# facebookresearch/SlowFast

Measured on AMD Instinct MI355X. Metric: clips/sec (fwd+bwd), SlowFast-8x8-R50 32x224^2 synthetic clips, per-GPU batch 32, higher is better.
Workload: dtype fp16; 1 GPU; SLOWFAST_8x8_R50: forward + cross_entropy loss + backward + sgd step, inputs resident in HBM, per-GPU batch 32; global_batch=32, parallelism=dp1, launch=hip-graph(fwd+bwd) + eager all-reduce/optimizer, optimizer=FlatOptimizer (fused unscale+norm+clip+update, dynamic loss scale on device)

## Files before the change

include/sfamd.h:

```cpp
#ifndef SFAMD_H
#define SFAMD_H
#include <stddef.h>
#include <stdint.h>
#ifdef __cplusplus
extern "C" {
#endif

#define SF_ABI_VERSION 32
typedef void* sf_stream_t;

typedef struct sf_conv_desc {
    int32_t N, Ci, Ti, Hi, Wi;
    int32_t Co, To, Ho, Wo;
    int32_t kT, kH, kW;
    int32_t sT, sH, sW;
    int32_t pT, pH, pW;
    int32_t dT, dH, dW;
    int32_t Cw;
    int32_t ldx, ldy;
    int32_t Cow;
} sf_conv_desc;

int sf_abi_version(void);
const char* sf_backend(void);
#define SF_ACT_FP16 0
#define SF_ACT_BF16_ID 1
int sf_act_dtype(void);
const char* sf_last_error(void);
const char* sf_build_id(void);

int sf_conv_weight_ld(const sf_conv_desc* d, int32_t* ldf, int32_t* ldd);
int sf_prep_weights(const sf_conv_desc* d, const float* w, void* wf, void* wd, sf_stream_t stream);
typedef struct sf_prep_item {
    const float* w;
    void* wf;
    void* wd;
    int32_t Co, Cow, Cw, Cp, taps, ldf, ldd;
    int32_t pad;
} sf_prep_item;
int sf_prep_item_fill(const sf_conv_desc* d, const float* w, void* wf, void* wd, sf_prep_item* item);
int64_t sf_prep_item_blocks(const sf_prep_item* item);
int sf_prep_weights_batch(const sf_prep_item* items, const int32_t* blk_item, const int32_t* blk_off, int32_t nblocks,
                          sf_stream_t stream);
int sf_conv_fwd_mtiles(const sf_conv_desc* d);
int sf_conv_fwd(const sf_conv_desc* d, const void* x, const void* wf, const float* in_scale, const float* in_shift,
                int in_relu, const float* bias, void* y, float* stat_part, sf_stream_t stream);
int sf_conv_fwd_fused(const sf_conv_desc* d, const void* x, const void* wf, const float* bias, const void* resid,
                      int32_t ldr, int out_relu, void* y, sf_stream_t stream);
int sf_conv_dgrad(const sf_conv_desc* d, const void* dy, const void* wd, const void* resid, int32_t ldr,
                  const void* resid_bits, void* dx, sf_stream_t stream);
int sf_conv_dgrad_bn(const sf_conv_desc* d, const void* dy, const void* wd, const void* resid, int32_t ldr,
                     const void* resid_bits, void* dx, const float* mask_scale, const float* mask_shift,
                     const void* mask_bits, const void* bn_y, int32_t bn_ldy, float* bn_part, int32_t bn_part_rows,
                     int32_t* bn_rows, sf_stream_t stream);
int64_t sf_conv_wgrad_workspace(const sf_conv_desc* d);
int64_t sf_conv_wgrad_rowtab_bytes(const sf_conv_desc* d);
int sf_conv_wgrad_rowtab(const sf_conv_desc* d, void* tab, sf_stream_t stream);
int sf_conv_wgrad(const sf_conv_desc* d, const void* x, const float* in_scale, const float* in_shift, int in_relu,
                  const void* dy, float* dw, float out_scale, int zero_first, void* workspace, int64_t workspace_bytes,
                  const void* rowtab, sf_stream_t stream);
int sf_conv_c_bwd_plan(const sf_conv_desc* d, int in_affine, int mask_bits, int32_t* tile_rows, int64_t* workspace_bytes);
int sf_conv_c_bwd(const sf_conv_desc* d, const void* dz, int32_t lddz, const void* mask_bits, const void* yc, int32_t ldyc,
                  const float* coef, const void* act, const void* wd, const float* bn_scale, const float* bn_shift,
                  const void* bn_y, int32_t bn_ldy, float* bn_part, int32_t bn_part_rows, int32_t* bn_rows, void* d_in,
                  int32_t ld_in, float* dw, float out_scale, int zero_first, void* workspace, int64_t workspace_bytes,
                  sf_stream_t stream);

int sf_bn_finalize(float* part, int32_t nblk, int32_t C, int32_t Creal, float count, const float* gamma, const float* beta,
                   float* running_mean, float* running_var, float momentum, float eps, float* scale, float* shift,
                   float* save_mean, float* save_rstd, sf_stream_t stream);
int sf_bn_act(int64_t M, int32_t C, const void* y, int32_t ldy, const float* scale, const float* shift, const void* r,
              int32_t ldr, const float* rscale, const float* rshift, int relu, void* out, int32_t ldo, void* mask_out,
              sf_stream_t stream);
int sf_bn_bwd_blocks(int64_t M, int32_t C);
int sf_bn_bwd_reduce(int64_t M, int32_t C, const void* dz, int32_t lddz, const void* zmask, int32_t ldm, const void* y,
                     int32_t ldy, const float* scale, const float* shift, int relu_self, float* part,
                     sf_stream_t stream);
int sf_bn_bwd_finalize(float* part, int32_t nblk, int32_t C, int32_t Creal, float count, const float* gamma, const float* mean,
                       const float* rstd, float inv_loss_scale, float* dgamma, float* dbeta, int accumulate,
                       float* coef, sf_stream_t stream);
int sf_bn_bwd_apply(int64_t M, int32_t C, const void* dz, int32_t lddz, const void* zmask, int32_t ldm, const void* y,
                    int32_t ldy, const float* scale, const float* shift, int relu_self, const float* coef, void* dy,
                    int32_t lddy, void* gout, int32_t ldg, sf_stream_t stream);

int sf_pool_fwd(int32_t N, int32_t T, int32_t H, int32_t W, int32_t C, int32_t kH, int32_t kW, int32_t sH, int32_t sW,
                int32_t pH, int32_t pW, const void* y, int32_t ldy, const float* scale, const float* shift, int relu,
                void* out, int32_t ldo, void* argmax, int32_t cls, sf_stream_t stream);
int sf_pool_bwd(int32_t N, int32_t T, int32_t H, int32_t W, int32_t C, int32_t kH, int32_t kW, int32_t sH, int32_t sW,
                int32_t pH, int32_t pW, const void* pooled, int32_t ldp, const void* argmax, int relu,
                const void* dout, int32_t lddo, void* g, int32_t ldg, int32_t cls, sf_stream_t stream);

int sf_pool3d_fwd(int32_t N, int32_t T, int32_t H, int32_t W, int32_t C, int32_t kT, int32_t kH, int32_t kW, const void* x,
                  int32_t ldx, void* out, int32_t ldo, void* argmax, sf_stream_t stream);
int sf_pool3d_bwd(int32_t N, int32_t T, int32_t H, int32_t W, int32_t C, int32_t kT, int32_t kH, int32_t kW,
                  const void* argmax, const void* dout, int32_t lddo, void* dx, int32_t lddx, sf_stream_t stream);

int sf_ncthw_to_cl(const float* x, int32_t N, int32_t C, int64_t S, int32_t Cp, void* out, sf_stream_t stream);
int sf_cl_to_ncthw(const void* x, int32_t ld, int32_t N, int32_t C, int64_t S, float* out, sf_stream_t stream);


int sf_bgemm(int64_t M, int32_t N, int32_t K, const void* A, int32_t lda, const void* W, int32_t ldw, const float* bias,
             const void* resid, int32_t ldr, void* Y, int32_t ldy, int32_t nbatch, int32_t bh, int64_t sa_b, int64_t sa_h,
             int64_t sw_b, int64_t sw_h, int64_t sy_b, int64_t sy_h, int64_t sr_b, int64_t sr_h, int32_t resid_row0,
             float alpha, sf_stream_t stream);
typedef struct sf_rows32 {
    const float* in;
    float* out;
    int32_t ld, period;
} sf_rows32;
int sf_gemm_rows32(int64_t M, int32_t N, int32_t K, const void* A, int32_t lda, const void* W, int32_t ldw, const float* bias,
                   const void* resid, int32_t ldr, void* Y, int32_t ldy, const sf_rows32* side, sf_stream_t stream);
int sf_bgemm_tn(int64_t M, int32_t R, int32_t Kc, const void* P, int32_t ldp, const void* X, int32_t ldx, void* Out,
                int32_t ldo, float scale, int32_t nbatch, int32_t bh, int64_t sp_b, int64_t sp_h, int64_t sx_b,
                int64_t sx_h, int64_t so_b, int64_t so_h, sf_stream_t stream);

int sf_layernorm_fwd(int64_t M, int32_t C, const void* x, int32_t ldx, const float* gamma, const float* beta, float eps,
                     void* y, int32_t ldy, float* mean, float* rstd, sf_stream_t stream);
int sf_layernorm_fwd_rows32(int64_t M, int32_t C, const void* x, int32_t ldx, const float* gamma, const float* beta, float eps,
                            void* y, int32_t ldy, float* mean, float* rstd, const sf_rows32* side, sf_stream_t stream);
int sf_layernorm_bwd_blocks(int64_t M, int32_t C);
int sf_layernorm_bwd(int64_t M, int32_t C, const void* dy, int32_t lddy, const void* x, int32_t ldx, const float* gamma,
                     const float* mean, const float* rstd, const void* resid, int32_t ldr, void* dx, int32_t lddx,
                     float* part, sf_stream_t stream);
int sf_layernorm_bwd_sums(int64_t M, int32_t C, const void* dy, int32_t lddy, const void* x, int32_t ldx, const float* gamma,
                          const float* mean, const float* rstd, const void* resid, int32_t ldr, void* dx, int32_t lddx,
                          float* part, sf_stream_t stream);
int sf_colsum_blocks(int64_t M, int32_t C);
int sf_colsum(int64_t M, int32_t C, const void* x, int32_t ldx, float* part, sf_stream_t stream);
int sf_colsum_finalize(float* part, int32_t nblk, int32_t C, int32_t fold, float* out0, float* out1, float scale,
                       int accumulate, sf_stream_t stream);
typedef struct sf_colfin_item {
    float* part;
    int32_t nblk, C, fold;
    float* out0;
    float* out1;
    float scale;
    int32_t accumulate;
    int32_t row_stride;
} sf_colfin_item;
int sf_colsum_finalize_batch(const sf_colfin_item* items, int32_t n, sf_stream_t stream);
int sf_rows_sum(const float* part, int32_t nblk, int64_t row_len, int64_t offset, int32_t n, float* out, float scale,
                int accumulate, sf_stream_t stream);
int sf_gelu_fwd(int64_t n, const void* h, void* a, sf_stream_t stream);
int sf_gelu_bwd(int64_t n, const void* h, const void* da, void* dh, sf_stream_t stream);

typedef struct sf_dw_desc {
    int32_t N, C, Cw, cls;
    int32_t Ti, Hi, Wi, To, Ho, Wo;
    int32_t kT, kH, kW, sT, sH, sW, pT, pH, pW;
    int32_t ldx, ldy;
    int32_t Cwreal;
} sf_dw_desc;
int sf_dwconv_fwd_blocks(const sf_dw_desc* d);
int sf_dwconv_fwd_sample_rows(const sf_dw_desc* d);
int sf_dwconv_fwd(const sf_dw_desc* d, const void* x, const float* w, void* y, float* stat_part, sf_stream_t stream);
int sf_dwconv_dgrad(const sf_dw_desc* d, const void* dy, const float* w, void* dx, sf_stream_t stream);
int sf_dwconv_dgrad_sum_rows(const sf_dw_desc* d);
int sf_dwconv_dgrad_sums(const sf_dw_desc* d, const void* dy, const float* w, void* dx, float* sum_part, sf_stream_t stream);
int64_t sf_dwconv_wgrad_workspace(const sf_dw_desc* d);
int sf_dwconv_wgrad(const sf_dw_desc* d, const void* x, const void* dy, float* dw, float out_scale, int zero_first,
                    void* workspace, int64_t workspace_bytes, sf_stream_t stream);
int sf_dwconv_pair_ok(const sf_dw_desc* d);
int sf_dwconv_fwd_pair(const sf_dw_desc* d, const void* x, const void* x2, const float* w, const float* w2, void* y, void* y2,
                       sf_stream_t stream);
int sf_dwconv_dgrad_pair(const sf_dw_desc* d, const void* dy, const void* dy2, const float* w, const float* w2, void* dx, void* dx2,
                         sf_stream_t stream);
int sf_dwconv_wgrad_pair(const sf_dw_desc* d, const void* x, const void* x2, const void* dy, const void* dy2, float* dw, float* dw2,
                         float out_scale, int zero_first, int zero_first2, void* workspace, int64_t workspace_bytes,
                         sf_stream_t stream);

typedef struct sf_attn_desc {
    int32_t B, heads, D, cls;
    int32_t Nq, qT, qH, qW;
    int32_t Nk, kT, kH, kW;
    int32_t rows_h, rows_w, rows_t;
} sf_attn_desc;
int sf_relpos_gather(const sf_attn_desc* d, const void* G, int32_t ldg, const int32_t* idx_h, const int32_t* idx_w,
                     const int32_t* idx_t, float* rq, sf_stream_t stream);
int sf_relpos_scatter(const sf_attn_desc* d, const float* drq, const int32_t* idx_h, const int32_t* idx_w,
                      const int32_t* idx_t, void* E, int32_t lde, sf_stream_t stream);
int sf_relpos_pack(const float* rel_h, const float* rel_w, const float* rel_t, int32_t rows_h, int32_t rows_w, int32_t rows_t,
                   int32_t D, int32_t TRp, void* t16, void* t16t, sf_stream_t stream);
int sf_relpos_unpack(const float* dtab, int32_t rows_h, int32_t rows_w, int32_t rows_t, int32_t D, float* grad_h, float* grad_w,
                     float* grad_t, int32_t acc_h, int32_t acc_w, int32_t acc_t, sf_stream_t stream);
int sf_softmax_fwd(const sf_attn_desc* d, void* s, int32_t lds, float scale, const float* rq, sf_stream_t stream);
int sf_softmax_bwd(const sf_attn_desc* d, void* dp, const void* prob, int32_t lds, float scale, float* drq,
                   sf_stream_t stream);
int sf_attn_fwd(const sf_attn_desc* d, const void* q, int32_t ldq, const void* k, const void* v, int32_t ldk, float scale,
                const float* rq, const void* onehot, int32_t residual, void* o, int32_t ldo, float* lse,
                sf_stream_t stream);
int64_t sf_attn_bwd_workspace(const sf_attn_desc* d);
int sf_attn_bwd(const sf_attn_desc* d, const void* q, int32_t ldq, const void* k, const void* v, int32_t ldk, float scale,
                const float* rq, const void* onehot, int32_t residual, const void* o, const void* dout, int32_t ldo,
                const float* lse, float* delta, void* dq, int32_t lddq, void* dk, void* dv, int32_t lddk, float* drq,
                void* workspace, int64_t workspace_bytes, sf_stream_t stream);
int sf_tmean_fwd(int32_t B, int32_t T, int64_t HW, int32_t C, const void* x, int32_t ldx, float* m, sf_stream_t stream);
int sf_tmean_bwd(int32_t B, int32_t T, int64_t HW, int32_t C, const float* dm, void* dx, int32_t lddx, sf_stream_t stream);
int sf_roi_align_max_fwd(int32_t R, int32_t B, int32_t H, int32_t W, int32_t C, int32_t res, float scale, int32_t aligned,
                         const float* m, const float* rois, float* out, int32_t ldo, int32_t col0, void* argmax,
                         sf_stream_t stream);
int sf_roi_align_max_bwd(int32_t R, int32_t B, int32_t H, int32_t W, int32_t C, int32_t res, float scale, int32_t aligned,
                         const float* rois, const float* dout, int32_t lddo, int32_t col0, const void* argmax, float* dm,
                         sf_stream_t stream);
int sf_gemm_act(int64_t M, int32_t N, int32_t K, const void* A, int32_t lda, const void* W, int32_t ldw, const float* bias,
                void* Y, int32_t ldy, int32_t mode, void* aux, int32_t ldaux, sf_stream_t stream);
int sf_gemm_act_colsum(int64_t M, int32_t N, int32_t K, const void* A, int32_t lda, const void* W, int32_t ldw,
                       const float* bias, void* Y, int32_t ldy, int32_t mode, void* aux, int32_t ldaux,
                       float* colsum_part, int32_t colsum_part_rows, int32_t* colsum_rows, sf_stream_t stream);
int sf_pack_clip_u8(const void* frames, int32_t N, int32_t Tin, int32_t H, int32_t W, const int32_t* t_index, int32_t Tout,
                    float mean0, float mean1, float mean2, float std0, float std1, float std2, int32_t reverse, void* out,
                    sf_stream_t stream);
int sf_mix_clip_f32(const float* src, float* dst, int32_t B, int32_t C, int32_t T, int32_t H, int32_t W, int32_t mode,
                    float lam, float one_minus_lam, int32_t yl, int32_t yh, int32_t xl, int32_t xh, sf_stream_t stream);
int sf_pack_clip_u8_mix(const void* frames, int32_t N, int32_t Tin, int32_t H, int32_t W, const int32_t* t_index, int32_t Tout,
                        float mean0, float mean1, float mean2, float std0, float std1, float std2, int32_t reverse, void* out,
                        int32_t mode, float lam, float one_minus_lam, int32_t yl, int32_t yh, int32_t xl, int32_t xh,
                        sf_stream_t stream);
int sf_mix_targets(const int64_t* labels, int32_t B, int32_t K, float on_value, float off_value, float lam, float one_minus_lam,
                   float* out, sf_stream_t stream);
// ... 108 lines not shown
```

slowfast_amd/csrc/sf_api.hip:

```cpp
#include "../../include/sfamd.h"
#include "sf_bn.h"
#include "sf_common.h"
#include "sf_igemm.h"
#include "sf_igemm2.h"
#include "sf_wgrad2.h"
#include "sf_cbwd.h"
#include "sf_pool.h"
#include "sf_dwconv.h"
#include "sf_dwsweep.h"
#include "sf_dwtemporal.h"
#include "sf_tokens.h"
#include "sf_x3d.h"
#include "sf_stem.h"
#include "sf_attn.h"
#include "sf_roi.h"
#include "sf_optim.h"
#include "sf_mixup.h"
#include "sf_erase.h"
#include "sf_pack.h"
#include "sf_sample.h"
#include "sf_color.h"
#include "sf_randaug.h"
#include "sf_hog.h"
#include "sf_pixel.h"

#include <stdarg.h>
#include <stdio.h>
#include <stdlib.h>
#include <string.h>

static thread_local char g_err[512] = "";

static int fail(const char* fmt, ...) {
    va_list ap;
    va_start(ap, fmt);
    vsnprintf(g_err, sizeof(g_err), fmt, ap);
    va_end(ap);
    return -1;
}
static int check_launch(const char* what) {
    hipError_t e = hipGetLastError();
    if (e != hipSuccess) return fail("%s: launch failed: %s", what, hipGetErrorString(e));
    return 0;
}
#define REQUIRE(cond, ...) \
    do { if (!(cond)) return fail(__VA_ARGS__); } while (0)

static inline int cdiv(int64_t a, int64_t b) { return (int)((a + b - 1) / b); }
static inline int roundup(int a, int b) { return (a + b - 1) / b * b; }

static inline int test_hook(const char* name, int def) { const char* e = getenv(name); return e ? atoi(e) : def; }
#ifdef SF_DIAG
static inline int tune_knob(const char* name, int def) { const char* e = getenv(name); return e ? atoi(e) : def; }
#else
#define tune_knob(name, def) (def)
#endif

extern "C" int sf_abi_version(void) { return SF_ABI_VERSION; }
extern "C" const char* sf_backend(void) {
#ifdef SF_HOSTSIM
    return "hostsim";
#else
    return "gfx950";
#endif
}
extern "C" int sf_act_dtype(void) { return SF_ACT_DTYPE_ID; }
extern "C" const char* sf_last_error(void) { return g_err; }
#ifndef SF_BUILD_ID
#define SF_BUILD_ID "unversioned"
#endif
extern "C" const char* sf_build_id(void) {
    static const char tagged[] = "sfamd-build-id:" SF_BUILD_ID;
    return tagged + 15;
}

static int check_desc(const sf_conv_desc* d) {
    REQUIRE(d != nullptr, "conv: null descriptor");
    REQUIRE(d->N > 0 && d->Ci > 0 && d->Co > 0, "conv: empty tensor");
    REQUIRE(d->Ci % 8 == 0 && d->Co % 8 == 0, "conv: channel counts must be multiples of 8 (Ci=%d Co=%d)", d->Ci, d->Co);
    REQUIRE(d->ldx >= d->Ci && d->ldx % 8 == 0 && d->ldy >= d->Co && d->ldy % 8 == 0, "conv: bad row pitch");
    REQUIRE(d->Cw > 0 && d->Cw <= d->Ci, "conv: Cw must be in (0, Ci]");
    REQUIRE(d->Cow >= 0 && d->Cow <= d->Co, "conv: Cow must be in [0, Co]");
    REQUIRE(d->sT > 0 && d->sH > 0 && d->sW > 0 && d->dT > 0 && d->dH > 0 && d->dW > 0, "conv: stride/dilation");
    int To = (d->Ti + 2 * d->pT - d->dT * (d->kT - 1) - 1) / d->sT + 1;
    int Ho = (d->Hi + 2 * d->pH - d->dH * (d->kH - 1) - 1) / d->sH + 1;
    int Wo = (d->Wi + 2 * d->pW - d->dW * (d->kW - 1) - 1) / d->sW + 1;
    REQUIRE(d->To >= 1 && d->Ho >= 1 && d->Wo >= 1 && d->To <= To && d->Ho <= Ho && d->Wo <= Wo,
            "conv: output dims (%d,%d,%d) exceed the geometry's (%d,%d,%d)", d->To, d->Ho, d->Wo, To, Ho, Wo);
    int64_t Mo = (int64_t)d->N * d->To * d->Ho * d->Wo, Mi = (int64_t)d->N * d->Ti * d->Hi * d->Wi;
    REQUIRE(Mo < (1ll << 31) && Mi < (1ll << 31), "conv: more than 2^31 positions");
    return 0;
}

static void fill_gather_common(GatherSide& g, const sf_conv_desc* d) {
    g.kT = d->kT; g.kH = d->kH; g.kW = d->kW;
    g.strT = d->sT; g.strH = d->sH; g.strW = d->sW;
    g.padT = d->pT; g.padH = d->pH; g.padW = d->pW;
    g.dilT = d->dT; g.dilH = d->dH; g.dilW = d->dW;
    g.fdkW = make_fastdiv(d->kW);
    g.fdkH = make_fastdiv(d->kH);
    g.fdsT = make_fastdiv(d->sT);
    g.fdsH = make_fastdiv(d->sH);
    g.fdsW = make_fastdiv(d->sW);
    g.scale = nullptr; g.shift = nullptr; g.relu = 0;
    g.fdHW = make_fastdiv((uint32_t)d->Hi * (uint32_t)d->Wi);
}
static bool is_pointwise(const sf_conv_desc* d) {
    return d->kH == 1 && d->kW == 1 && d->sT == 1 && d->sH == 1 && d->sW == 1 && d->pH == 0 && d->pW == 0 &&
           d->Ho == d->Hi && d->Wo == d->Wi;
}

static GatherSide gather_fwd(const sf_conv_desc* d, const void* x, const float* sc, const float* sh, int relu) {
    GatherSide g;
    memset(&g, 0, sizeof(g));
    fill_gather_common(g, d);
    g.src = (const f16*)x; g.ld = d->ldx; g.C = d->Ci;
    g.sT = d->Ti; g.sH = d->Hi; g.sW = d->Wi;
    g.mode = 0;
    g.Ktot = d->kT * d->kH * d->kW * d->Ci;
    g.fdC = make_fastdiv(d->Ci);
    g.fdrW = make_fastdiv(d->Wo); g.fdrH = make_fastdiv(d->Ho); g.fdrT = make_fastdiv(d->To);
    g.rowT = d->To;
    g.scale = sc; g.shift = sh; g.relu = relu;
    return g;
}
static GatherSide gather_dgrad(const sf_conv_desc* d, const void* dy) {
    GatherSide g;
    memset(&g, 0, sizeof(g));
    fill_gather_common(g, d);
    g.src = (const f16*)dy; g.ld = d->ldy; g.C = d->Co;
    g.sT = d->To; g.sH = d->Ho; g.sW = d->Wo;
    g.mode = 1;
    g.Ktot = d->kT * d->kH * d->kW * d->Co;
    g.fdC = make_fastdiv(d->Co);
    g.fdrW = make_fastdiv(d->Wi); g.fdrH = make_fastdiv(d->Hi); g.fdrT = make_fastdiv(d->Ti);
    g.rowT = d->Ti;
    return g;
}

static bool igemm_glds_ok(const IgemmParams& p, bool pw) {
    static const bool off = tune_knob("SF_IGEMM_GLDS", 1) == 0;
    if (off || !pw || p.g.scale) return false;
    if (p.g.Ktot != p.g.C || p.g.Ktot % 32 != 0 || p.g.ld % 8 != 0 || p.ldw % 8 != 0) return false;
    if (p.g.padT != 0) return false;
    if (((uintptr_t)p.g.src | (uintptr_t)p.wmat) & 15) return false;
    if (p.bh > 0 && ((p.sa_b | p.sa_h | p.sw_b | p.sw_h) & 7)) return false;
    return true;
}

static inline bool sf_trace() { return test_hook("SF_TRACE", 0) != 0; }

enum GemmKind { GEMM_GEN1, GEMM_GEN2, GEMM_GEN2_CLASSES };
struct GemmPlan {
    GemmKind kind;
    bool pw;
    int nbatch;
    int bn, bk;
    bool t128;
    bool glds, cap;
// ... 629 lines not shown
            }
    hipLaunchKernelGGL(sf_wgrad2_rowtab_kernel, dim3(cdiv(t.M, SF_THREADS)), dim3(SF_THREADS), 0, s, t);
}

extern "C" int64_t sf_conv_wgrad_rowtab_bytes(const sf_conv_desc* d) {
    if (check_desc(d)) return -1;
    return (int64_t)plan_conv_wgrad(d, false).tab_bytes;
}

extern "C" int sf_conv_wgrad_rowtab(const sf_conv_desc* d, void* tab, sf_stream_t stream) {
    if (check_desc(d)) return -1;
    REQUIRE(tab && (uintptr_t)tab % 16 == 0, "sf_conv_wgrad_rowtab: tab must be a 16-byte aligned device pointer");
    REQUIRE(plan_conv_wgrad(d, false).path == WGRAD_ROWTAB, "sf_conv_wgrad_rowtab: this geometry does not take the row-table kernel (sf_conv_wgrad_rowtab_bytes == 0)");
    launch_rowtab(d, tab, (hipStream_t)stream);
    return check_launch("wgrad_rowtab");
}

extern "C" int64_t sf_conv_wgrad_workspace(const sf_conv_desc* d) {
    if (check_desc(d)) return -1;
    const int64_t plain = (int64_t)plan_conv_wgrad(d, false).ws_bytes, affine = (int64_t)plan_conv_wgrad(d, true).ws_bytes;
    return plain > affine ? plain : affine;
}

extern "C" int sf_conv_wgrad(const sf_conv_desc* d, const void* x, const float* in_scale, const float* in_shift,
                             int in_relu, const void* dy, float* dw, float out_scale, int zero_first,
                             void* workspace, int64_t workspace_bytes, const void* rowtab, sf_stream_t stream) {
    if (check_desc(d)) return -1;
    REQUIRE(x && dy && dw && workspace, "sf_conv_wgrad: null pointer");
    REQUIRE((in_scale == nullptr) == (in_shift == nullptr), "sf_conv_wgrad: in_scale/in_shift must come together");
    REQUIRE(!in_scale || d->Ci <= 512, "sf_conv_wgrad: fused input BatchNorm supports Ci <= 512 (got %d)", d->Ci);
    hipStream_t s = (hipStream_t)stream;
    GatherSide gk = gather_fwd(d, x, in_scale, in_shift, in_relu);
    const WgradPlan w = plan_conv_wgrad(d, in_scale != nullptr);
    REQUIRE(workspace_bytes >= (int64_t)w.ws_bytes, "sf_conv_wgrad: workspace too small (%lld < %lld bytes)",
            (long long)workspace_bytes, (long long)w.ws_bytes);
    float* slabs = (float*)((char*)workspace + w.tab_bytes);
    if (w.path == WGRAD_ROWTAB) {
        REQUIRE(((uintptr_t)x | (uintptr_t)dy | (uintptr_t)workspace) % 16 == 0, "sf_conv_wgrad: operands must be 16-byte aligned");
        Wgrad2Params q;
        memset(&q, 0, sizeof(q));
        int ti = 0;
        for (int kt = 0; kt < d->kT; ++kt)
            for (int kh = 0; kh < d->kH; ++kh)
                for (int kw = 0; kw < d->kW; ++kw, ++ti) q.dlin[ti] = (kt * d->dT * d->Hi + kh * d->dH) * d->Wi + kw * d->dW;
        if (!rowtab) launch_rowtab(d, workspace, s);
        else REQUIRE((uintptr_t)rowtab % 16 == 0, "sf_conv_wgrad: rowtab must be 16-byte aligned");
        q.x = (const f16*)x; q.ldx = d->ldx; q.C = d->Ci;
        q.dy = (const f16*)dy; q.ldy = d->ldy; q.Co = d->Co;
        q.M = d->N * d->To * d->Ho * d->Wo; q.Ktot = gk.Ktot;
        q.rowtab = (const i32x2*)(rowtab ? rowtab : workspace);
        q.ws = slabs; q.Co_pad = w.Co_pad; q.Kpad = w.Kpad;
        q.tiles_k = w.tiles_k; q.tiles_c = w.tiles_c; q.rows_per_split = w.rows_per_split;
        q.stage_stride = (w.thin && tune_knob("SF_WGRAD2T_RR", 1) != 0) ? w.splits : 0;
        const dim3 grid((unsigned)(w.tiles_k * w.tiles_c * w.slabs));
        if (sf_trace()) fprintf(stderr, "[sfamd] wgrad2: M=%d Co=%d K=%d tiles %dx%d splits %d%s\n", q.M, q.Co, q.Ktot, w.tiles_c, w.tiles_k, w.splits,
                                w.dual ? " (two per workgroup)" : "");
        if (w.thin) {
            if (w.BMW == 16 && w.BKW == 128) hipLaunchKernelGGL((sf_wgrad2t_kernel<16, 128, 2>), grid, dim3(256), 0, s, q);
            else if (w.BMW == 32 && w.BKW == 128) hipLaunchKernelGGL((sf_wgrad2t_kernel<32, 128, 2>), grid, dim3(256), 0, s, q);
            else if (w.BMW == 16) hipLaunchKernelGGL((sf_wgrad2t_kernel<16, 32, 3>), grid, dim3(256), 0, s, q);
            else hipLaunchKernelGGL((sf_wgrad2t_kernel<32, 32, 3>), grid, dim3(256), 0, s, q);
        } else if (w.dual) {
            if (w.BMW == 128) hipLaunchKernelGGL((sf_wgrad2_kernel<128, true>), grid, dim3(1024), 0, s, q);
            else hipLaunchKernelGGL((sf_wgrad2_kernel<64, true>), grid, dim3(1024), 0, s, q);
        } else {
            if (w.BMW == 128) hipLaunchKernelGGL((sf_wgrad2_kernel<128>), grid, dim3(512), 0, s, q);
            else hipLaunchKernelGGL((sf_wgrad2_kernel<64>), grid, dim3(512), 0, s, q);
        }
    } else if (w.path == WGRAD_STEM) {
        const StemPlan& sp = w.stem;
        StemParams q = stem_params(d, sp, x);
        q.dy = (const f16*)dy; q.ws = (float*)workspace;
        if (sf_trace()) fprintf(stderr, "[sfamd] stem_wgrad: %d workgroups x %d tiles\n", sp.wg_blocks, sp.tiles_per_block);
        static const bool stem_plain = tune_knob("SF_STEM_XCD", 1) == 0;
        q.plain_order = stem_plain ? 1 : 0;
        const dim3 grid(sp.wg_blocks), block(SF_STEM_WG_THREADS);
        if (d->Co <= 8 && sp.small) hipLaunchKernelGGL((sf_stem_wgrad_kernel<8, SF_STEM_CHUNKS_SMALL>), grid, block, 0, s, q);
        else if (d->Co <= 8) hipLaunchKernelGGL((sf_stem_wgrad_kernel<8, SF_STEM_CHUNKS>), grid, block, 0, s, q);
        else if (sp.small) hipLaunchKernelGGL((sf_stem_wgrad_kernel<16, SF_STEM_CHUNKS_SMALL>), grid, block, 0, s, q);
        else hipLaunchKernelGGL((sf_stem_wgrad_kernel<16, SF_STEM_CHUNKS>), grid, block, 0, s, q);
    } else {
        REQUIRE(w.splits <= 65535, "sf_conv_wgrad: too many splits");
        WgradParams p;
        memset(&p, 0, sizeof(p));
        p.g = gk;
        p.dy = (const f16*)dy; p.ldy = d->ldy; p.Co = d->Co;
        p.M = d->N * d->To * d->Ho * d->Wo;
        p.ws = (float*)workspace; p.Co_pad = w.Co_pad; p.Kpad = w.Kpad;
        p.nchunks = w.nchunks; p.chunks_per_split = w.chunks_per_split;
        launch_wgrad1(w.BMW, p, dim3(w.tiles_k, w.tiles_c, w.splits), s);
    }
    if (check_launch("wgrad")) return -1;
    launch_wgrad_reduce(d, slabs, w.slabs, w.Co_pad, w.Kpad, w.path == WGRAD_STEM && w.stem.thin3, dw, out_scale, zero_first, s);
    return check_launch("wgrad_reduce");
}

struct CbwdPlan {
    bool ok;
    int cip, cop, R;
    size_t ws_bytes;
};
#define SF_CBWD_MAX_WGS 1024
template <int CIP, int COP>
static void cbwd_fill(CbwdPlan& w) {
    using K = CbwdCfg<CIP, COP>;
    w.R = K::R;
    w.ws_bytes = (size_t)SF_CBWD_MAX_WGS * COP * CIP * 4;
}
#define SF_CBWD_FOR_SHAPE(cip, cop, ...)                                                         \
    do {                                                                                         \
        if ((cip) == 16 && (cop) == 32) { constexpr int CIP_ = 16, COP_ = 32; __VA_ARGS__; }            \
        else if ((cip) == 16 && (cop) == 64) { constexpr int CIP_ = 16, COP_ = 64; __VA_ARGS__; }       \
        else if ((cip) == 16 && (cop) == 128) { constexpr int CIP_ = 16, COP_ = 128; __VA_ARGS__; }     \
        else if ((cip) == 16 && (cop) == 256) { constexpr int CIP_ = 16, COP_ = 256; __VA_ARGS__; }     \
        else if ((cip) == 32 && (cop) == 32) { constexpr int CIP_ = 32, COP_ = 32; __VA_ARGS__; }       \
        else if ((cip) == 32 && (cop) == 64) { constexpr int CIP_ = 32, COP_ = 64; __VA_ARGS__; }       \
        else if ((cip) == 32 && (cop) == 128) { constexpr int CIP_ = 32, COP_ = 128; __VA_ARGS__; }     \
        else if ((cip) == 32 && (cop) == 256) { constexpr int CIP_ = 32, COP_ = 256; __VA_ARGS__; }     \
        else if ((cip) == 64 && (cop) == 32) { constexpr int CIP_ = 64, COP_ = 32; __VA_ARGS__; }       \
        else if ((cip) == 64 && (cop) == 64) { constexpr int CIP_ = 64, COP_ = 64; __VA_ARGS__; }       \
        else if ((cip) == 64 && (cop) == 128) { constexpr int CIP_ = 64, COP_ = 128; __VA_ARGS__; }     \
        else { constexpr int CIP_ = 64, COP_ = 256; __VA_ARGS__; }                                      \
    } while (0)
static CbwdPlan plan_cbwd(const sf_conv_desc* d, bool in_affine, bool mask_bits) {
    CbwdPlan w;
    memset(&w, 0, sizeof(w));
    if (test_hook("SF_CBWD", 1) == 0) return w;
    if (d->kT != 1 || d->kH != 1 || d->kW != 1 || d->sT != 1 || d->sH != 1 || d->sW != 1 || d->pT || d->pH || d->pW) return w;
    if (d->To != d->Ti || d->Ho != d->Hi || d->Wo != d->Wi) return w;
    if (d->Ci % 8 || d->Ci > 64 || d->Co % 32 || d->Co > 256) return w;
    if (in_affine || !mask_bits) return w;
    w.cip = d->Ci <= 16 ? 16 : d->Ci <= 32 ? 32 : 64;
    w.cop = d->Co <= 32 ? 32 : d->Co <= 64 ? 64 : d->Co <= 128 ? 128 : 256;
    SF_CBWD_FOR_SHAPE(w.cip, w.cop, (cbwd_fill<CIP_, COP_>(w)));
    w.ok = true;
    return w;
}

extern "C" int sf_conv_c_bwd_plan(const sf_conv_desc* d, int in_affine, int mask_bits, int32_t* tile_rows,
                                  int64_t* workspace_bytes) {
    if (check_desc(d)) return -1;
    const CbwdPlan w = plan_cbwd(d, in_affine != 0, mask_bits != 0);
    if (tile_rows) *tile_rows = w.ok ? 128 : 0;
    if (workspace_bytes) *workspace_bytes = w.ok ? (int64_t)w.ws_bytes : 0;
    return w.ok ? 1 : 0;
}

extern "C" int sf_conv_c_bwd(const sf_conv_desc* d, const void* dz, int32_t lddz, const void* mask_bits, const void* yc,
                             int32_t ldyc, const float* coef, const void* act, const void* wd, const float* bn_scale,
                             const float* bn_shift, const void* bn_y, int32_t bn_ldy, float* bn_part, int32_t bn_part_rows,
                             int32_t* bn_rows, void* d_in, int32_t ld_in, float* dw, float out_scale, int zero_first,
                             void* workspace, int64_t workspace_bytes, sf_stream_t stream) {
    if (check_desc(d)) return -1;
    REQUIRE(dz && mask_bits && yc && coef && act && wd && d_in && dw && workspace, "sf_conv_c_bwd: null pointer");
    const CbwdPlan w = plan_cbwd(d, false, true);
    REQUIRE(w.ok, "sf_conv_c_bwd: this geometry keeps sf_bn_bwd_apply + sf_conv_wgrad + sf_conv_dgrad_bn (sf_conv_c_bwd_plan == 0)");
    REQUIRE(lddz >= d->Co && lddz % 8 == 0 && ldyc >= d->Co && ldyc % 8 == 0 && ld_in >= d->Ci && ld_in % 8 == 0,
            "sf_conv_c_bwd: bad row pitch");
    REQUIRE((((uintptr_t)dz | (uintptr_t)yc | (uintptr_t)act | (uintptr_t)wd | (uintptr_t)d_in | (uintptr_t)workspace) & 15) == 0,
            "sf_conv_c_bwd: operands must be 16-byte aligned");
    REQUIRE(workspace_bytes >= (int64_t)w.ws_bytes, "sf_conv_c_bwd: workspace too small (%lld < %lld bytes)",
            (long long)workspace_bytes, (long long)w.ws_bytes);
    const int64_t M = (int64_t)d->N * d->Ti * d->Hi * d->Wi;
    const int ntiles = cdiv(M, 128);
    const bool fuse = bn_part != nullptr;
    if (fuse) {
        REQUIRE(bn_scale && bn_shift && bn_y && bn_rows, "sf_conv_c_bwd: the fused reduction needs bn_scale, bn_shift, bn_y and bn_rows");
        REQUIRE(bn_ldy >= d->Ci && bn_ldy % 8 == 0 && ((uintptr_t)bn_y & 15) == 0, "sf_conv_c_bwd: bad bn_y pitch / alignment");
        REQUIRE(bn_part_rows >= ntiles, "sf_conv_c_bwd: the partial table needs ceil(positions / tile_rows) rows of [2][Ci] floats");
    }
    int32_t ldf, ldd;
    sf_conv_weight_ld(d, &ldf, &ldd);
    CbwdParams p;
    memset(&p, 0, sizeof(p));
    p.M = (int)M; p.Ci = d->Ci; p.Co = d->Co;
    p.dz = (const f16*)dz; p.lddz = lddz; p.bits = (const uint8_t*)mask_bits; p.yc = (const f16*)yc; p.ldyc = ldyc;
    p.coef = coef; p.act = (const f16*)act; p.ldact = d->ldx; p.wd = (const f16*)wd; p.ldw = ldd;
    if (fuse) { p.bnb_y = (const f16*)bn_y; p.bnb_ld = bn_ldy; p.bnb_scale = bn_scale; p.bnb_shift = bn_shift; p.bnb_part = bn_part; }
    p.dx = (f16*)d_in; p.lddx = ld_in; p.ws = (float*)workspace; p.tiles128 = ntiles;
    int wgs;
    const WgradPlan w2 = plan_conv_wgrad(d, false);
    const int forced = test_hook("SF_CBWD_WGS", 0);
    if (forced > 0) {
        wgs = forced < SF_CBWD_MAX_WGS ? forced : SF_CBWD_MAX_WGS;
        p.rps = roundup(cdiv(M, wgs), 32);
        wgs = cdiv(M, p.rps);
    } else if (w2.path == WGRAD_ROWTAB && w2.thin && w2.splits <= SF_CBWD_MAX_WGS) {
        wgs = w2.splits; p.rps = 0;
    } else {
        const WgradPlan w1 = plan_wgrad1(d);
        wgs = w1.splits; p.rps = w1.chunks_per_split * 32;
        REQUIRE(wgs <= SF_CBWD_MAX_WGS, "sf_conv_c_bwd: %d splits", wgs);
    }
    hipStream_t s = (hipStream_t)stream;
    SF_CBWD_FOR_SHAPE(w.cip, w.cop, hipLaunchKernelGGL((sf_cbwd_kernel<CIP_, COP_>), dim3(wgs), dim3(SF_THREADS), 0, s, p));
    if (check_launch("conv_c_bwd")) return -1;
    if (bn_rows) *bn_rows = fuse ? ntiles : 0;
    launch_wgrad_reduce(d, (const float*)workspace, wgs, w.cop, w.cip, false, dw, out_scale, zero_first, s);
    return check_launch("conv_c_bwd_reduce");
}

static RowTile make_rowtile(int64_t M, int C, int max_blocks, dim3& grid) {
    RowTile rt;
    rt.M = (int)M; rt.C = C;
    const int G = C / 8;
    const int TG = G < SF_THREADS ? G : SF_THREADS;
    const int rpi = SF_THREADS / TG;
    int passes = cdiv(M, (int64_t)rpi * max_blocks);
    if (passes < 1) passes = 1;
    rt.rows_per_block = rpi * passes;
    grid = dim3(cdiv(M, rt.rows_per_block), cdiv(G, SF_THREADS));
    return rt;
}
static int check_rows(const char* who, int64_t M, int C) {
    REQUIRE(M > 0 && M < (1ll << 31), "%s: bad row count", who);
    REQUIRE(C > 0 && C % 8 == 0, "%s: C must be a positive multiple of 8 (got %d)", who, C);
    return 0;
}

static const int kFoldAbove = tune_knob("SF_FOLD_ABOVE", 2048);
static int fold_partials(float* part, int& nblk, int C, hipStream_t s) {
    if (nblk <= kFoldAbove || nblk <= 256) return 1;
    const int group = nblk <= 2048 ? 16 : nblk <= 8192 ? 32 : 64;
    const int cols = 2 * C;
    dim3 grid(cdiv(cols, SF_THREADS), cdiv(nblk, group));
    hipLaunchKernelGGL(sf_part_fold_kernel, grid, dim3(SF_THREADS), 0, s, part, nblk, cols, group);
    nblk = cdiv(nblk, group);
    return group;
}

extern "C" int sf_bn_finalize(float* part, int32_t nblk, int32_t C, int32_t Creal, float count, const float* gamma,
                              const float* beta, float* running_mean, float* running_var, float momentum, float eps,
                              float* scale, float* shift, float* save_mean, float* save_rstd, sf_stream_t stream) {
    REQUIRE(gamma && beta && scale && shift, "sf_bn_finalize: null pointer");
    REQUIRE(nblk > 0 ? part != nullptr : (running_mean && running_var), "sf_bn_finalize: missing statistics source");
    REQUIRE(Creal > 0 && Creal <= C, "sf_bn_finalize: Creal must be in (0, C]");
    BnFinalizeParams p;
    p.row_stride = nblk > 0 ? fold_partials(part, nblk, C, (hipStream_t)stream) : 1;
    p.part = part; p.nblk = nblk; p.C = C; p.Creal = Creal; p.count = count; p.gamma = gamma; p.beta = beta;
    p.running_mean = running_mean; p.running_var = running_var; p.momentum = momentum; p.eps = eps;
    p.scale = scale; p.shift = shift; p.save_mean = save_mean; p.save_rstd = save_rstd;
    hipLaunchKernelGGL(sf_bn_finalize_kernel, dim3(cdiv(C, SF_FIN_CH)), dim3(sf_fin_threads(p.nblk)), 0, (hipStream_t)stream, p);
    return check_launch("bn_finalize");
}

extern "C" int sf_bn_act(int64_t M, int32_t C, const void* y, int32_t ldy, const float* scale, const float* shift,
                         const void* r, int32_t ldr, const float* rscale, const float* rshift, int relu, void* out,
                         int32_t ldo, void* mask_out, sf_stream_t stream) {
    if (check_rows("sf_bn_act", M, C)) return -1;
    REQUIRE(y && out, "sf_bn_act: null pointer");
    BnActParams p;
    dim3 grid;
    p.rt = make_rowtile(M, C, 8192, grid);
    p.y = (const f16*)y; p.ldy = ldy; p.scale = scale; p.shift = shift;
    p.r = (const f16*)r; p.ldr = ldr; p.rscale = rscale; p.rshift = rshift;
    p.relu = relu; p.out = (f16*)out; p.ldo = ldo; p.mask_out = (uint8_t*)mask_out;
    hipLaunchKernelGGL(sf_bn_act_kernel, grid, dim3(SF_THREADS), 0, (hipStream_t)stream, p);
    return check_launch("bn_act");
}

static const int kBwdBlocks = tune_knob("SF_BN_BWD_BLOCKS", 1024);
extern "C" int sf_bn_bwd_blocks(int64_t M, int32_t C) {
    if (check_rows("sf_bn_bwd_blocks", M, C)) return -1;
    dim3 grid;
    make_rowtile(M, C, kBwdBlocks, grid);
    return (int)grid.x;
}

extern "C" int sf_bn_bwd_reduce(int64_t M, int32_t C, const void* dz, int32_t lddz, const void* zmask, int32_t ldm,
                                const void* y, int32_t ldy, const float* scale, const float* shift, int relu_self,
                                float* part, sf_stream_t stream) {
    if (check_rows("sf_bn_bwd_reduce", M, C)) return -1;
    REQUIRE(dz && y && part, "sf_bn_bwd_reduce: null pointer");
    REQUIRE(!relu_self || (scale && shift), "sf_bn_bwd_reduce: relu_self needs scale/shift");
    BnBwdReduceParams p;
    dim3 grid;
    p.rt = make_rowtile(M, C, kBwdBlocks, grid);
    p.dz = (const f16*)dz; p.lddz = lddz; p.zmask = (const f16*)zmask; p.ldm = ldm;
    p.y = (const f16*)y; p.ldy = ldy; p.scale = scale; p.shift = shift; p.relu_self = relu_self; p.part = part;
    hipLaunchKernelGGL(sf_bn_bwd_reduce_kernel, grid, dim3(SF_THREADS), 0, (hipStream_t)stream, p);
    return check_launch("bn_bwd_reduce");
}

extern "C" int sf_bn_bwd_finalize(float* part, int32_t nblk, int32_t C, int32_t Creal, float count, const float* gamma,
                                  const float* mean, const float* rstd, float inv_loss_scale, float* dgamma,
                                  float* dbeta, int accumulate, float* coef, sf_stream_t stream) {
    REQUIRE(part && gamma && mean && rstd && dgamma && dbeta && coef, "sf_bn_bwd_finalize: null pointer");
    BnBwdFinalizeParams p;
    p.row_stride = fold_partials(part, nblk, C, (hipStream_t)stream);
    REQUIRE(Creal > 0 && Creal <= C, "sf_bn_bwd_finalize: Creal must be in (0, C]");
    p.part = part; p.nblk = nblk; p.C = C; p.Creal = Creal; p.count = count; p.gamma = gamma; p.mean = mean; p.rstd = rstd;
    p.inv_loss_scale = inv_loss_scale; p.dgamma = dgamma; p.dbeta = dbeta; p.accumulate = accumulate; p.coef = coef;
    hipLaunchKernelGGL(sf_bn_bwd_finalize_kernel, dim3(cdiv(C, SF_FIN_CH)), dim3(sf_fin_threads(p.nblk)), 0, (hipStream_t)stream, p);
    return check_launch("bn_bwd_finalize");
}

extern "C" int sf_bn_bwd_apply(int64_t M, int32_t C, const void* dz, int32_t lddz, const void* zmask, int32_t ldm,
                               const void* y, int32_t ldy, const float* scale, const float* shift, int relu_self,
                               const float* coef, void* dy, int32_t lddy, void* gout, int32_t ldg,
                               sf_stream_t stream) {
    if (check_rows("sf_bn_bwd_apply", M, C)) return -1;
    REQUIRE(dz && y && coef && dy, "sf_bn_bwd_apply: null pointer");
    REQUIRE(!relu_self || (scale && shift), "sf_bn_bwd_apply: relu_self needs scale/shift");
    BnBwdApplyParams p;
    dim3 grid;
    p.rt = make_rowtile(M, C, 8192, grid);
    p.dz = (const f16*)dz; p.lddz = lddz; p.zmask = (const f16*)zmask; p.ldm = ldm;
    p.y = (const f16*)y; p.ldy = ldy; p.scale = scale; p.shift = shift; p.relu_self = relu_self;
    p.coef = coef; p.dy = (f16*)dy; p.lddy = lddy; p.gout = (f16*)gout; p.ldg = ldg;
    p.sample_add = nullptr; p.fdS = make_fastdiv(1);
    hipLaunchKernelGGL(sf_bn_bwd_apply_kernel, grid, dim3(SF_THREADS), 0, (hipStream_t)stream, p);
    return check_launch("bn_bwd_apply");
}
extern "C" int sf_bn_bwd_apply_sample(int64_t M, int32_t C, const void* dz, int32_t lddz, const void* y, int32_t ldy,
                                      const float* coef, const float* sample_add, int64_t S, void* dy, int32_t lddy,
                                      sf_stream_t stream) {
    if (check_rows("sf_bn_bwd_apply_sample", M, C)) return -1;
    REQUIRE(dz && y && coef && dy && sample_add, "sf_bn_bwd_apply_sample: null pointer");
    REQUIRE(S > 0 && S < (1ll << 31) && M % S == 0, "sf_bn_bwd_apply_sample: rows must be whole samples of S positions");
    BnBwdApplyParams p;
    dim3 grid;
    p.rt = make_rowtile(M, C, 8192, grid);
    p.dz = (const f16*)dz; p.lddz = lddz; p.zmask = nullptr; p.ldm = 0;
    p.y = (const f16*)y; p.ldy = ldy; p.scale = nullptr; p.shift = nullptr; p.relu_self = 0;
    p.coef = coef; p.dy = (f16*)dy; p.lddy = lddy; p.gout = nullptr; p.ldg = 0;
    p.sample_add = sample_add; p.fdS = make_fastdiv((uint32_t)S);
    hipLaunchKernelGGL(sf_bn_bwd_apply_kernel, grid, dim3(SF_THREADS), 0, (hipStream_t)stream, p);
    return check_launch("bn_bwd_apply_sample");
}

static int fill_pool(PoolParams& p, int32_t N, int32_t T, int32_t H, int32_t W, int32_t C, int32_t kH, int32_t kW,
                     int32_t sH, int32_t sW, int32_t pH, int32_t pW, const void* y, int32_t ldy, const float* scale,
                     const float* shift, int relu) {
    REQUIRE(C > 0 && C % 8 == 0, "pool: C must be a multiple of 8");
    REQUIRE((scale == nullptr) == (shift == nullptr), "pool: scale/shift must come together");
    memset(&p, 0, sizeof(p));
    p.y = (const f16*)y; p.ldy = ldy; p.scale = scale; p.shift = shift; p.relu = relu;
    p.N = N; p.T = T; p.H = H; p.W = W; p.C = C;
    p.kH = kH; p.kW = kW; p.sH = sH; p.sW = sW; p.pH = pH; p.pW = pW;
    p.Ho = (H + 2 * pH - kH) / sH + 1;
    p.Wo = (W + 2 * pW - kW) / sW + 1;
    p.fdG = make_fastdiv(C / 8);
    return 0;
}
static int pool_grid(int64_t total) {
    int64_t b = (total + SF_THREADS - 1) / SF_THREADS;
    return (int)(b > 65536 ? 65536 : b);
}

extern "C" int sf_pool_fwd(int32_t N, int32_t T, int32_t H, int32_t W, int32_t C, int32_t kH, int32_t kW, int32_t sH,
                           int32_t sW, int32_t pH, int32_t pW, const void* y, int32_t ldy, const float* scale,
                           const float* shift, int relu, void* out, int32_t ldo, void* argmax, int32_t cls,
                           sf_stream_t stream) {
    PoolParams p;
    if (fill_pool(p, N, T, H, W, C, kH, kW, sH, sW, pH, pW, y, ldy, scale, shift, relu)) return -1;
    REQUIRE(y && out, "sf_pool_fwd: null pointer");
    p.cls = cls ? 1 : 0; p.fdT = make_fastdiv(T);
    REQUIRE(kH * kW <= 255, "sf_pool_fwd: window too large for the byte argmax");
    p.out = (f16*)out; p.ldo = ldo; p.argmax = (uint8_t*)argmax;
    p.fdW = make_fastdiv(p.Wo); p.fdH = make_fastdiv(p.Ho);
    p.total = (int64_t)N * T * p.Ho * p.Wo * (C / 8);
    REQUIRE(p.total < (1ll << 31), "sf_pool_fwd: too many elements");
    hipLaunchKernelGGL(sf_pool_fwd_kernel, dim3(pool_grid(p.total + (int64_t)N * (C / 8))), dim3(SF_THREADS), 0,
                       (hipStream_t)stream, p);
    return check_launch("pool_fwd");
}

extern "C" int sf_pool_bwd(int32_t N, int32_t T, int32_t H, int32_t W, int32_t C, int32_t kH, int32_t kW, int32_t sH,
                           int32_t sW, int32_t pH, int32_t pW, const void* pooled, int32_t ldp, const void* argmax,
                           int relu, const void* dout, int32_t lddo, void* g, int32_t ldg, int32_t cls,
                           sf_stream_t stream) {
    PoolParams p;
    if (fill_pool(p, N, T, H, W, C, kH, kW, sH, sW, pH, pW, nullptr, 0, nullptr, nullptr, relu)) return -1;
    REQUIRE(argmax && dout && g, "sf_pool_bwd: null pointer");
    (void)pooled; (void)ldp;
    p.cls = cls ? 1 : 0; p.fdT = make_fastdiv(T);
    p.out = (f16*)g; p.ldo = ldg; p.dout = (const f16*)dout; p.lddo = lddo;
    p.pooled = (const f16*)pooled; p.ldp = ldp; p.argmax = (uint8_t*)argmax;
    p.fdW = make_fastdiv(W); p.fdH = make_fastdiv(H);
    p.total = (int64_t)N * T * H * W * (C / 8);
    REQUIRE(p.total < (1ll << 31), "sf_pool_bwd: too many elements");
    p.fdsH = make_fastdiv(sH); p.fdsW = make_fastdiv(sW);
    if (kH <= 2 * sH && kW <= 2 * sW)
        hipLaunchKernelGGL(sf_pool_bwd4_kernel, dim3(pool_grid(p.total + (int64_t)N * (C / 8))), dim3(SF_THREADS), 0,
                           (hipStream_t)stream, p);
    else
        hipLaunchKernelGGL(sf_pool_bwd_kernel, dim3(pool_grid(p.total + (int64_t)N * (C / 8))), dim3(SF_THREADS), 0,
                           (hipStream_t)stream, p);
    return check_launch("pool_bwd");
}

extern "C" int sf_pool3d_fwd(int32_t N, int32_t T, int32_t H, int32_t W, int32_t C, int32_t kT, int32_t kH, int32_t kW,
                             const void* x, int32_t ldx, void* out, int32_t ldo, void* argmax, sf_stream_t stream) {
    REQUIRE(x && out && argmax && C > 0 && C % 8 == 0 && kT > 0 && kH > 0 && kW > 0 && kT * kH * kW <= 255,
            "sf_pool3d_fwd: bad arguments");
    Pool3dParams p;
    p.N = N; p.T = T; p.H = H; p.W = W; p.C = C; p.kT = kT; p.kH = kH; p.kW = kW;
    p.To = T / kT; p.Ho = H / kH; p.Wo = W / kW;
    REQUIRE(p.To > 0 && p.Ho > 0 && p.Wo > 0, "sf_pool3d_fwd: window larger than the input");
    p.x = (const f16*)x; p.ldx = ldx; p.out = (f16*)out; p.ldo = ldo; p.argmax = (uint8_t*)argmax;
    p.dout = nullptr; p.lddo = 0;
    p.fdG = make_fastdiv(C / 8); p.fdW = make_fastdiv(p.Wo); p.fdH = make_fastdiv(p.Ho); p.fdT = make_fastdiv(p.To);
    p.total = (int64_t)N * p.To * p.Ho * p.Wo * (C / 8);
    REQUIRE(p.total < (1ll << 31), "sf_pool3d_fwd: too many elements");
    hipLaunchKernelGGL(sf_pool3d_fwd_kernel, dim3(pool_grid(p.total)), dim3(SF_THREADS), 0, (hipStream_t)stream, p);
    return check_launch("pool3d_fwd");
}
extern "C" int sf_pool3d_bwd(int32_t N, int32_t T, int32_t H, int32_t W, int32_t C, int32_t kT, int32_t kH, int32_t kW,
                             const void* argmax, const void* dout, int32_t lddo, void* dx, int32_t lddx, sf_stream_t stream) {
    REQUIRE(argmax && dout && dx && C > 0 && C % 8 == 0 && kT > 0 && kH > 0 && kW > 0, "sf_pool3d_bwd: bad arguments");
    Pool3dParams p;
    p.N = N; p.T = T; p.H = H; p.W = W; p.C = C; p.kT = kT; p.kH = kH; p.kW = kW;
    p.To = T / kT; p.Ho = H / kH; p.Wo = W / kW;
    p.x = nullptr; p.ldx = 0; p.out = (f16*)dx; p.ldo = lddx; p.argmax = (uint8_t*)argmax;
    p.dout = (const f16*)dout; p.lddo = lddo;
    p.fdG = make_fastdiv(C / 8); p.fdW = make_fastdiv(W); p.fdH = make_fastdiv(H); p.fdT = make_fastdiv(T);
    p.total = (int64_t)N * T * H * W * (C / 8);
    REQUIRE(p.total < (1ll << 31), "sf_pool3d_bwd: too many elements");
    hipLaunchKernelGGL(sf_pool3d_bwd_kernel, dim3(pool_grid(p.total)), dim3(SF_THREADS), 0, (hipStream_t)stream, p);
    return check_launch("pool3d_bwd");
}

extern "C" int sf_ncthw_to_cl(const float* x, int32_t N, int32_t C, int64_t S, int32_t Cp, void* out,
                              sf_stream_t stream) {
    REQUIRE(x && out && (Cp % 8 == 0 || Cp == 4) && Cp >= C, "sf_ncthw_to_cl: bad arguments");
    static const bool quad = test_hook("SF_LAYOUT_QUAD", 1) != 0;
    if (quad && C <= 4 && Cp <= 8 && S % 4 == 0 && (((uintptr_t)x | (uintptr_t)out) & 15) == 0) {
        const int grid = pool_grid((int64_t)N * (S / 4));
        if (Cp == 4) hipLaunchKernelGGL(sf_ncthw_to_cl_quad_kernel<4>, dim3(grid), dim3(SF_THREADS), 0, (hipStream_t)stream, x, (f16*)out, N, C, S / 4);
        else hipLaunchKernelGGL(sf_ncthw_to_cl_quad_kernel<8>, dim3(grid), dim3(SF_THREADS), 0, (hipStream_t)stream, x, (f16*)out, N, C, S / 4);
        return check_launch("ncthw_to_cl");
    }
    hipLaunchKernelGGL(sf_ncthw_to_cl_kernel, dim3(pool_grid((int64_t)N * S)), dim3(SF_THREADS), 0,
                       (hipStream_t)stream, x, (f16*)out, N, C, S, Cp);
// ... 2022 lines not shown
```

slowfast_amd/csrc/sf_cbwd.h:

```cpp
#pragma once
#include "sf_bn.h"
#include "sf_common.h"
#include "sf_igemm.h"

struct CbwdParams {
    int M, Ci, Co;
    const f16* dz; int lddz;
    const uint8_t* bits;
    const f16* yc; int ldyc;
    const float* coef;
    const f16* act; int ldact;
    const f16* wd; int ldw;
    const f16* bnb_y; int bnb_ld;
    const float* bnb_scale; const float* bnb_shift;
    float* bnb_part;
    f16* dx; int lddx;
    float* ws;
    int rps;
    int tiles128;
};

template <int CIP, int COP>
struct CbwdCfg {
    static constexpr int R = COP >= 128 ? 64 : 128;
    static constexpr int NSUB = 128 / R;
    static constexpr int NJ = CIP / 16, KS = COP / 32, TI = R / 64;
    static constexpr int WAVES_M = COP == 32 ? 4 : 1, WAVES_C = 4 / WAVES_M;
    static constexpr int TC = COP / 16 / WAVES_C;
    static constexpr int KSM = R / WAVES_M / 32;
    static constexpr int LDY = COP + 8;
    static constexpr int CGO = COP / 8, RPP = SF_THREADS / CGO, NCH = R / RPP;
    static constexpr int ACH = CIP / 8, NACT = R * ACH / 64;
    static constexpr int NEPI = (R * ACH + SF_THREADS - 1) / SF_THREADS;
    static constexpr int DY_ELEMS = R * LDY, ACT_ELEMS = R * CIP, WD_ELEMS = CIP * LDY;
    static constexpr int RED_ELEMS = 4 * ACH * 24 * 2;
    static constexpr int UNION_ELEMS = DY_ELEMS > ACT_ELEMS + RED_ELEMS ? DY_ELEMS : ACT_ELEMS + RED_ELEMS;
    static constexpr int LDS_ELEMS = UNION_ELEMS + ACT_ELEMS + WD_ELEMS + 3 * COP * 2 + 2 * CIP * 2;
    static_assert(WAVES_M == 1 || LDS_ELEMS * 2 >= 4 * (COP / 16) * NJ * 256 * 4, "the cross-wave sum reuses the tile buffers");
    static constexpr int LDS_BYTES = LDS_ELEMS * 2;
    static constexpr int HELD = 4 * NJ * (TI + TC) + 9 * NCH + 4 * NEPI;
    static constexpr int OCC = HELD <= 72 ? 3 : 2;
    static_assert(R % 64 == 0 && R % RPP == 0 && NACT >= 1 && (R * ACH) % 64 == 0, "tile shape");
    static_assert(SF_THREADS % ACH == 0 && 64 % ACH == 0, "a thread keeps one d_in column group");
};

template <int CIP, int COP>
__global__ __launch_bounds__(SF_THREADS, (CbwdCfg<CIP, COP>::OCC)) void sf_cbwd_kernel(CbwdParams p) {
    using K = CbwdCfg<CIP, COP>;
    constexpr int R = K::R, LDY = K::LDY, NJ = K::NJ, TI = K::TI, TC = K::TC;
    __shared__ __attribute__((aligned(16))) f16 smem[K::LDS_ELEMS];
    f16* const DyL = smem;
    f16* const StL = smem;
    float* const red = reinterpret_cast<float*>(smem + K::ACT_ELEMS);
    f16* const ActL = smem + K::UNION_ELEMS;
    f16* const WdL = ActL + K::ACT_ELEMS;
    float* const coefL = reinterpret_cast<float*>(WdL + K::WD_ELEMS);
    float* const bnL = coefL + 3 * COP;

    const int tid = threadIdx.x;
    const int lane = tid & 63, wave = __builtin_amdgcn_readfirstlane(tid >> 6);
    const int pl = lane & 15, g4 = lane >> 4;
    const int G = (int)gridDim.x;
    const f16* const zline = reinterpret_cast<const f16*>(sf_zero_line);
    const bool bnb = p.bnb_part != nullptr;

    for (int q = tid; q < CIP * K::CGO; q += SF_THREADS) {
        const int ci = q / K::CGO, cg = q % K::CGO;
        f16x8 v = zero8();
        if (ci < p.Ci && cg * 8 < p.Co) v = ld16(p.wd + (int64_t)ci * p.ldw + cg * 8);
        st16(WdL + ci * LDY + cg * 8, v);
    }
    for (int q = tid; q < 3 * COP; q += SF_THREADS) {
        const int k = q / COP, c = q % COP;
        coefL[q] = c < p.Co ? p.coef[k * p.Co + c] : 0.f;
    }
    for (int q = tid; q < 2 * CIP; q += SF_THREADS) {
        const int k = q / CIP, c = q % CIP;
        bnL[q] = (bnb && c < p.Ci) ? (k ? p.bnb_shift[c] : p.bnb_scale[c]) : (k ? 0.f : 1.f);
    }

    const int scg = tid % K::CGO, srow = tid / K::CGO;
    const bool scol_ok = scg * 8 < p.Co;
    const int scgc = scol_ok ? scg : 0;
    const int ecg = tid % K::ACH;
    const bool ecol_ok = ecg * 8 < p.Ci;
    const int ecgc = ecol_ok ? ecg : 0;

    int r0 = 0, r1 = p.M, T0 = (int)blockIdx.x, Tstep = G, nwalk = 0;
    if (p.rps > 0) {
        r0 = (int)blockIdx.x * p.rps;
        r1 = r0 + p.rps < p.M ? r0 + p.rps : p.M;
        T0 = r0 >> 7;
        Tstep = 1;
        if (r1 > r0) nwalk = (((r1 + 127) >> 7) - T0) * K::NSUB;
    } else if (T0 < p.tiles128) nwalk = ((p.tiles128 - 1 - T0) / G + 1) * K::NSUB;
    auto tile_m0 = [&](int q) { return (T0 + (q / K::NSUB) * Tstep) * 128 + (q % K::NSUB) * R; };

    f16x8 dzr[K::NCH], ycr[K::NCH], ybr[K::NEPI];
    uint32_t mbr[K::NCH];
    auto load_regs = [&](int m0) {
#pragma unroll
        for (int u = 0; u < K::NCH; ++u) {
            int m = m0 + srow + u * K::RPP;
            if (m > p.M - 1) m = p.M - 1;
            dzr[u] = ld16(p.dz + (int64_t)m * p.lddz + scgc * 8);
            ycr[u] = ld16(p.yc + (int64_t)m * p.ldyc + scgc * 8);
            mbr[u] = p.bits[(int64_t)m * (p.Co >> 3) + scgc];
        }
    };
    auto load_yb = [&](int m0) {
#pragma unroll
        for (int e = 0; e < K::NEPI; ++e) {
            int m = m0 + (tid + e * SF_THREADS) / K::ACH;
            if (m > p.M - 1) m = p.M - 1;
            ybr[e] = ld16(p.bnb_y + (int64_t)m * p.bnb_ld + ecgc * 8);
        }
    };
    auto issue_act = [&](int m0) {
#pragma unroll
        for (int j = 0; j < (K::NACT + 3) / 4; ++j) {
            const int q = wave + 4 * j;
            if (q < K::NACT) {
                const int c = q * 64 + lane;
                const int m = m0 + c / K::ACH, cc = c % K::ACH;
                const f16* g = (m >= r0 && m < r1 && cc * 8 < p.Ci) ? p.act + (int64_t)m * p.ldact + cc * 8 : zline;
                SF_GLOBAL_LOAD_LDS16_ASM(g, ActL + q * 512);
            }
        }
    };


    f32x4 wacc[TC][NJ];
#pragma unroll
    for (int i = 0; i < TC; ++i)
#pragma unroll
        for (int j = 0; j < NJ; ++j) wacc[i][j] = (f32x4){0.f, 0.f, 0.f, 0.f};
    const int wc = wave % K::WAVES_C, wm = wave / K::WAVES_C;
    const int cobase = wc * TC * 16, mbase = wm * (R / K::WAVES_M);
    const int rowbase = wave * (R / 4);

    float bsg[8], bsgy[8];
#pragma unroll
    for (int e = 0; e < 8; ++e) { bsg[e] = 0.f; bsgy[e] = 0.f; }
    const int nq = nwalk;
    if (nq > 0) { load_regs(tile_m0(0)); issue_act(tile_m0(0)); }
    for (int q = 0; q < nq; ++q) {
        const int m0 = tile_m0(q);
        const int T = T0 + (q / K::NSUB) * Tstep;
        const bool owner = T * 128 >= r0 && T * 128 < r1;
        const bool more = q + 1 < nq;
        SF_WAIT_VMEM();
        __syncthreads();
        {
            float k1[8], k2[8], k3[8];
#pragma unroll
            for (int e = 0; e < 8; ++e) { k1[e] = coefL[scg * 8 + e]; k2[e] = coefL[COP + scg * 8 + e]; k3[e] = coefL[2 * COP + scg * 8 + e]; }
#pragma unroll
            for (int u = 0; u < K::NCH; ++u) {
                const int row = srow + u * K::RPP;
                const uint32_t b = mbr[u];
                const f16x8 yv = ycr[u];
                float g[8];
#pragma unroll
                for (int e = 0; e < 8; ++e) g[e] = (float)dzr[u][e];
#pragma unroll
                for (int e = 0; e < 8; ++e) g[e] = ((b >> e) & 1u) ? g[e] : 0.f;
                f16x8 o;
#pragma unroll
                for (int e = 0; e < 8; ++e) o[e] = (f16)(k1[e] * g[e] + k2[e] + k3[e] * (float)yv[e]);
                if (!(scol_ok && m0 + row < p.M)) o = zero8();
                st16(DyL + row * LDY + scg * 8, o);
            }
        }
        __syncthreads();
        if (more) load_regs(tile_m0(q + 1));
#pragma unroll
        for (int ks = 0; ks < K::KSM; ++ks) {
            f16x8 af[TC], bf[NJ];
#pragma unroll
            for (int h = 0; h < 2; ++h) {
                const int m = mbase + ks * 32 + 8 * g4 + 4 * h + (pl >> 2);
#pragma unroll
                for (int i = 0; i < TC; ++i) {
                    const f16x4 v = as_f16x4(SF_LDS_TR16(DyL + m * LDY + cobase + i * 16 + 4 * (pl & 3)));
                    af[i][4 * h + 0] = v[0]; af[i][4 * h + 1] = v[1]; af[i][4 * h + 2] = v[2]; af[i][4 * h + 3] = v[3];
                }
#pragma unroll
                for (int j = 0; j < NJ; ++j) {
                    const f16x4 v = as_f16x4(SF_LDS_TR16(ActL + m * CIP + j * 16 + 4 * (pl & 3)));
                    bf[j][4 * h + 0] = v[0]; bf[j][4 * h + 1] = v[1]; bf[j][4 * h + 2] = v[2]; bf[j][4 * h + 3] = v[3];
                }
            }
#pragma unroll
            for (int i = 0; i < TC; ++i)
#pragma unroll
                for (int j = 0; j < NJ; ++j) wacc[i][j] = SF_MFMA16(af[i], bf[j], wacc[i][j]);
        }
        SF_BARRIER_KEEP_VMEM();
        if (more) issue_act(tile_m0(q + 1));
        if (!owner) continue;
        if (bnb) load_yb(m0);
        f32x4 dacc[TI][NJ];
#pragma unroll
        for (int i = 0; i < TI; ++i)
#pragma unroll
            for (int j = 0; j < NJ; ++j) dacc[i][j] = (f32x4){0.f, 0.f, 0.f, 0.f};
#pragma unroll
        for (int ks = 0; ks < K::KS; ++ks) {
            f16x8 bf[NJ];
#pragma unroll
            for (int j = 0; j < NJ; ++j) bf[j] = ld16(WdL + (j * 16 + pl) * LDY + ks * 32 + 8 * g4);
#pragma unroll
            for (int i = 0; i < TI; ++i) {
                const f16x8 af = ld16(DyL + (rowbase + i * 16 + pl) * LDY + ks * 32 + 8 * g4);
#pragma unroll
                for (int j = 0; j < NJ; ++j) dacc[i][j] = SF_MFMA16(af, bf[j], dacc[i][j]);
            }
        }
        SF_BARRIER_KEEP_VMEM();
#pragma unroll
        for (int i = 0; i < TI; ++i)
#pragma unroll
            for (int j = 0; j < NJ; ++j)
#pragma unroll
                for (int r = 0; r < 4; ++r) StL[(rowbase + i * 16 + 4 * g4 + r) * CIP + j * 16 + pl] = (f16)dacc[i][j][r];
        SF_BARRIER_KEEP_VMEM();
        float bsc[8], bsh[8];
#pragma unroll
        for (int e = 0; e < 8; ++e) { bsc[e] = bnL[ecg * 8 + e]; bsh[e] = bnL[CIP + ecg * 8 + e]; }
#pragma unroll
        for (int e = 0; e < K::NEPI; ++e) {
            const int idx = tid + e * SF_THREADS;
            const int row = idx / K::ACH, m = m0 + row;
            if (idx < R * K::ACH && m < p.M && ecol_ok) {
                const f16x8 v = ld16(StL + row * CIP + ecg * 8);
                st16(p.dx + (int64_t)m * p.lddx + ecg * 8, v);
                if (bnb) bnb_accumulate(v, ybr[e], bsc, bsh, bsg, bsgy, false, 0u);
            }
        }
        if (bnb && q % K::NSUB == K::NSUB - 1) {
            bnb_reduce_store<4, K::ACH>(bsg, bsgy, red, p.bnb_part + (int64_t)T * 2 * p.Ci, 0, p.Ci);
#pragma unroll
            for (int e = 0; e < 8; ++e) { bsg[e] = 0.f; bsgy[e] = 0.f; }
        }
    }

    float* slab = p.ws + (int64_t)blockIdx.x * (COP * CIP);
    if constexpr (K::WAVES_M == 4) {
        __syncthreads();
        float* rd = reinterpret_cast<float*>(smem);
#pragma unroll
        for (int i = 0; i < TC; ++i)
#pragma unroll
            for (int j = 0; j < NJ; ++j)
#pragma unroll
                for (int r = 0; r < 4; ++r) rd[(((wave * TC + i) * NJ + j) * 4 + r) * 64 + lane] = wacc[i][j][r];
        __syncthreads();
        constexpr int TE = TC * NJ * 256;
        for (int e = tid; e < TE; e += SF_THREADS) {
            const float v = (rd[e] + rd[TE + e]) + (rd[2 * TE + e] + rd[3 * TE + e]);
            const int ln = e & 63, r = (e >> 6) & 3, tt = e >> 8;
            const int i = tt / NJ, j = tt - i * NJ;
            slab[(i * 16 + 4 * (ln >> 4) + r) * CIP + j * 16 + (ln & 15)] = v;
        }
    } else {
#pragma unroll
        for (int i = 0; i < TC; ++i)
#pragma unroll
            for (int j = 0; j < NJ; ++j)
#pragma unroll
                for (int r = 0; r < 4; ++r) slab[(cobase + i * 16 + 4 * g4 + r) * CIP + j * 16 + pl] = wacc[i][j][r];
    }
}
```

slowfast_amd/engine.py:

```python
import functools
import os

import torch

from . import lib as _sflib

from . import ops

_f16 = _sflib.act_dtype()
_listeners = []
FORCE_WEIGHT_PREP = False
PARAM_EPOCH = 0
PACK_RECORD = None
PACK_PLAN = os.environ.get("SF_PACK_PLAN", "1") != "0"
BN_FUSE_REDUCE = os.environ.get("SF_BN_FUSE_REDUCE", "1") != "0"
CAT_IN_PLACE = os.environ.get("SF_CAT_IN_PLACE", "1") != "0"
SEGMENTS = None


class _Segments:
    def __init__(self):
        self.cuts = []

    def cut(self, tensors):
# ... 222 lines not shown
        bn.running_var.add_(bn.momentum * (var - bn.running_var))
    st = ops.bn_finalize(tot, total, bn.weight, bn.bias, None, None, bn.momentum, bn.eps, training=True, C=C)
    return BNState(*st)


def as_cl(t):
    if t.dtype == _f16 and ops.is_cl(t):
        return t
    return ops.to_cl(t)


GRADS_VIA_AUTOGRAD = False
_pending_grads = {}


def record_params(ctx, params):
    ctx._sf_params = params
    ctx._sf_via_autograd = GRADS_VIA_AUTOGRAD


def delivers_grads(backward):
    @functools.wraps(backward)
    def wrapped(ctx, *grads):
        global GRADS_VIA_AUTOGRAD
        prev = GRADS_VIA_AUTOGRAD
        GRADS_VIA_AUTOGRAD = getattr(ctx, "_sf_via_autograd", prev)
        try:
            return backward(ctx, *grads)
        finally:
            GRADS_VIA_AUTOGRAD = prev
    return wrapped


def _grad_dest(param):
    if GRADS_VIA_AUTOGRAD:
        g = _pending_grads.get(id(param))
        if g is not None:
            return g, False
        g = torch.empty_like(param, memory_format=torch.contiguous_format)
        _pending_grads[id(param)] = g
        return g, True
    if param.grad is not None:
        assert param.grad.dtype == torch.float32 and param.grad.is_contiguous()
        return param.grad, False
    g = torch.empty_like(param, memory_format=torch.contiguous_format)
    param.grad = g
    return g, True


def param_grads(ctx, lead, extra=()):
    n = len(ctx.needs_input_grad) - lead
    if not GRADS_VIA_AUTOGRAD:
        return ((None,) * n, (None,) * len(extra)) if extra else (None,) * n
    ps = getattr(ctx, "_sf_params", ())
    assert len(ps) == n, "Function.forward must record its *params (ctx._sf_params)"
    out = tuple(_pending_grads.pop(id(p), None) for p in ps)
    if extra:
        return out, tuple(_pending_grads.pop(id(p), None) for p in extra)
    return out


class BNState:
    __slots__ = ("scale", "shift", "mean", "rstd")

    def __init__(self, scale, shift, mean, rstd):
        self.scale, self.shift, self.mean, self.rstd = scale, shift, mean, rstd


class ConvUnit:

    def __init__(self, conv, bn=None):
        assert conv.groups == 1, "grouped convolutions are handled by the depthwise path, not the implicit GEMM"
        assert conv.padding_mode == "zeros"
        assert bn is None or bn.momentum is not None, "cumulative-average BatchNorm is not supported"
        self.conv, self.bn = conv, bn
        self._geoms = {}
        self._wkey, self._w, self._planned = None, None, False

    def geom(self, in_shape):
        key = tuple(in_shape)
        g = self._geoms.get(key)
        if g is None:
            c = self.conv
            g = ops.ConvGeom(key, c.out_channels, c.kernel_size, c.stride, c.padding, c.dilation, Cw=c.in_channels)
            self._geoms[key] = g
        return g

    def weights(self, geom, fresh=False):
        w = self.conv.weight
        key = (w.data_ptr(), w._version, geom.Ci, w.device, PARAM_EPOCH)
        if (fresh and FORCE_WEIGHT_PREP and not self._planned) or self._wkey != key:
            need_dgrad = geom.Ci - geom.Cw < 8
            self._w = ops.prep_weights(w.detach(), geom, need_dgrad=need_dgrad)
            self._wkey = key
            if PACK_RECORD is not None:
                PACK_RECORD.append((self, geom, need_dgrad))
        return self._w

    def pack_item(self, geom, need_dgrad):
        w = self.conv.weight
        wf = torch.empty((geom.Co, geom.ldf), dtype=_f16, device=w.device)
        wd = torch.empty((geom.Ci, geom.ldd), dtype=_f16, device=w.device) if need_dgrad else None
        return w, geom.desc(geom.Ci, geom.Co), wf, wd

    def pack_key(self, geom):
        w = self.conv.weight
        return (w.data_ptr(), w._version, geom.Ci, w.device, PARAM_EPOCH)

    def pack_assign(self, geom, wf, wd):
        self._w, self._wkey, self._planned = (wf, wd), self.pack_key(geom), True

    def forward(self, x, in_affine, training):
        geom = self.geom(x.shape)
        wf, _ = self.weights(geom, fresh=True)
        bn = self.bn
        if bn is None:
            y, _ = ops.conv_fwd(x, wf, geom, in_affine=in_affine, bias=self.conv.bias, stats=False)
            return y, None
        use_batch_stats = training or bn.running_mean is None
        y, part = ops.conv_fwd(x, wf, geom, in_affine=in_affine, bias=self.conv.bias, stats=use_batch_stats)
        return y, bn_statistics(bn, part, geom.out_rows, geom.Co, training)

    def backward(self, x, in_affine, dy, need_dx, resid=None, resid_bits=None, bn_fuse=None):
        geom = self.geom(x.shape)
        w = self.conv.weight
        if w.requires_grad:
            dw, zero_first = _grad_dest(w)
            ops.conv_wgrad(x, dy, geom, dw, in_affine=in_affine, out_scale=1.0, zero_first=zero_first)
        if not need_dx:
            return None
        _, wd = self.weights(geom)
        if bn_fuse is not None:
            if isinstance(bn_fuse, dict):
                return ops.conv_dgrad(dy, wd, geom, resid=resid, resid_bits=resid_bits, bn=bn_fuse)
            y, st = bn_fuse
            return ops.conv_dgrad(dy, wd, geom, resid=resid, bn=(y, st.scale, st.shift))
        return ops.conv_dgrad(dy, wd, geom, resid=resid, resid_bits=resid_bits)

    def _bn_grad_dest(self):
        bn = self.bn
        if bn.weight.requires_grad:
            dgamma, zg = _grad_dest(bn.weight)
            dbeta, zb = _grad_dest(bn.bias)
            assert zg == zb
            return dgamma, dbeta, not zg
        return torch.empty_like(bn.weight), torch.empty_like(bn.bias), False

    def fused_c_geom(self, x):
        if self.bn is None or _sync_of(self.bn) is not None or not self.conv.weight.requires_grad:
            return None
        geom = self.geom(x.shape)
        return geom if ops.conv_c_bwd_plan(geom) is not None else None

    def fused_c_backward(self, geom, x, dz, y, st, bits, part=None, bn_fuse=None):
        bn = self.bn
        dgamma, dbeta, accumulate = self._bn_grad_dest()
        coef = ops.bn_bwd_coef(dz, y, bn.weight, st.mean, st.rstd, dgamma, dbeta, zmask=bits, inv_loss_scale=1.0,
                               accumulate=accumulate, part=part)
        dw, zero_first = _grad_dest(self.conv.weight)
        _, wd = self.weights(geom)
        fuse = None
        if bn_fuse is not None:
            y0, st0 = bn_fuse
            fuse = (y0, st0.scale, st0.shift)
        return ops.conv_c_bwd(dz, bits, y, coef, x, wd, geom, dw, bn=fuse, out_scale=1.0, zero_first=zero_first)

    def bn_backward(self, dz, y, st, zmask=None, relu_self=False, want_g=False, part=None):
        bn = self.bn
        dgamma, dbeta, accumulate = self._bn_grad_dest()
        return ops.bn_bwd(dz, y, bn.weight, st.mean, st.rstd, dgamma, dbeta, zmask=zmask,
                          relu_affine=(st.scale, st.shift) if relu_self else None, inv_loss_scale=1.0,
                          accumulate=accumulate, want_g=want_g, sync=_sync_of(bn), part=part)

    def params(self):
        p = [self.conv.weight]
        if self.conv.bias is not None:
            p.append(self.conv.bias)
        if self.bn is not None:
            p += [self.bn.weight, self.bn.bias]
        return p

    def _fold_source(self, w):
        return w

    def fold(self):
        w = self.conv.weight.detach().float()
        b = self.conv.bias.detach().float() if self.conv.bias is not None else None
        bn = self.bn
        if bn is not None:
            assert bn.running_mean is not None, "BatchNorm without running statistics cannot be folded"
            scale = torch.rsqrt(bn.running_var.detach().float() + bn.eps)
            if bn.weight is not None:
                scale = scale * bn.weight.detach().float()
            shift = -bn.running_mean.detach().float() * scale
            if bn.bias is not None:
                shift = shift + bn.bias.detach().float()
            w = w * scale.view(-1, 1, 1, 1, 1)
            b = shift if b is None else b * scale + shift
        self._fold_w, self._fold_b, self._fold_packed = self._fold_source(w).contiguous(), b, {}

    def infer(self, x, relu=False, resid=None, out=None):
        geom = self.geom(x.shape)
        packed = self._fold_packed.get(geom.in_shape)
        if packed is None:
            wf, _ = ops.prep_weights(self._fold_w, geom, need_dgrad=False)
            b = self._fold_b
            if b is not None and b.numel() < geom.Co:
                b = torch.nn.functional.pad(b, (0, geom.Co - b.numel()))
            packed = self._fold_packed[geom.in_shape] = (wf, None if b is None else b.contiguous())
        return ops.conv_fwd_fused(x, packed[0], geom, bias=packed[1], resid=resid, relu=relu, out=out)


class StemConvUnit(ConvUnit):

    def __init__(self, conv, bn=None):
        super().__init__(conv, bn)
        kT, kH, kW = conv.kernel_size
        sT, sH, sW = conv.stride
        pT, pH, pW = conv.padding
        assert conv.in_channels <= 4 and sW % 2 == 0 and conv.dilation == (1, 1, 1)
        self.lead = pW % 2
        self.kext = kW + self.lead + ((kW + self.lead) % 2)
        self.k2 = (kT, kH, self.kext // 2)
        self.s2 = (sT, sH, sW // 2)
        self.p2 = (pT, pH, (pW + self.lead) // 2)

    def prepare_input(self, x):
        if getattr(x, "_sf_wpairs", False):
            return x
        return ops.ncthw_to_cl_wpairs(x.float())

    @staticmethod
    def prepare_shape(shape):
        N, C, T, H, W = shape
        return (N, 8, T, H, W // 2)

    def geom(self, in_shape):
        key = tuple(in_shape)
        g = self._geoms.get(key)
        if g is None:
            c = self.conv
            N, C2, T, H, W2 = key
            assert C2 == 8
            Wo = (2 * W2 + 2 * c.padding[2] - c.kernel_size[2]) // c.stride[2] + 1
            g = ops.ConvGeom(key, c.out_channels, self.k2, self.s2, self.p2, (1, 1, 1), Cw=8)
            g = ops.ConvGeom(key, c.out_channels, self.k2, self.s2, self.p2, (1, 1, 1), Cw=8,
                             out_dims=(g.To, g.Ho, Wo))
            self._geoms[key] = g
        return g

    def _virtual_weight(self, w):
        Co, Cin, kT, kH, kW = w.shape
        wv = torch.nn.functional.pad(w, (self.lead, self.kext - kW - self.lead, 0, 0, 0, 0, 0, 4 - Cin))
        wv = wv.view(Co, 4, kT, kH, self.kext // 2, 2).permute(0, 5, 1, 2, 3, 4)
        return wv.reshape(Co, 8, kT, kH, self.kext // 2).contiguous()

    def _fold_source(self, w):
        return self._virtual_weight(w)

    def weights(self, geom, fresh=False):
        w = self.conv.weight
        key = (w.data_ptr(), w._version, geom.Ci, w.device, PARAM_EPOCH)
        if (fresh and FORCE_WEIGHT_PREP) or self._wkey != key:
            self._w = ops.prep_weights(self._virtual_weight(w.detach()), geom, need_dgrad=False)
            self._wkey = key
        return self._w

    def backward(self, x, in_affine, dy, need_dx, resid=None):
        assert not need_dx, "the stems take the input clip: no data gradient"
        geom = self.geom(x.shape)
        w = self.conv.weight
        if w.requires_grad:
            Co, Cin, kT, kH, kW = w.shape
            dwv = torch.empty((Co, 8, kT, kH, self.kext // 2), dtype=torch.float32, device=w.device)
            ops.conv_wgrad(x, dy, geom, dwv, in_affine=in_affine, out_scale=1.0, zero_first=True)
            dw = dwv.view(Co, 2, 4, kT, kH, self.kext // 2).permute(0, 2, 3, 4, 5, 1).reshape(Co, 4, kT, kH, self.kext)
            dw = dw[:, :Cin, :, :, self.lead:self.lead + kW]
            dst, zero_first = _grad_dest(w)
            if zero_first:
                dst.copy_(dw)
            else:
                dst.add_(dw)
        return None


class StemFn(torch.autograd.Function):

    @staticmethod
    def forward(ctx, x, mod, *params):
        record_params(ctx, params)
        unit = mod._unit
        xcl = unit.prepare_input(x) if isinstance(unit, StemConvUnit) else ops.to_cl(x)
        y, st = unit.forward(xcl, None, mod.training)
        k, s, p = mod.pool_layer.kernel_size, mod.pool_layer.stride, mod.pool_layer.padding
        assert k[0] == 1 and s[0] == 1 and p[0] == 0, "stem pooling is spatial-only in every reference config"
        out, arg = ops.pool_fwd(y, k[1:], s[1:], p[1:], affine=(st.scale, st.shift, True))
        if CAPTURE is not None:
            CAPTURE.append({"kind": "stem", "mod": mod, "raw": [y], "bn": [(st.scale, st.shift)], "out": out,
                            "argmax": torch.where(arg == 255, torch.zeros_like(arg), arg)})
        ctx.mod, ctx.xcl, ctx.y, ctx.st = mod, xcl, y, st
        ctx.pool = (tuple(k[1:]), tuple(s[1:]), tuple(p[1:]))
        ctx.pooled, ctx.arg = out, arg
        return out

    @staticmethod
    @delivers_grads
    def backward(ctx, dout):
        unit = ctx.mod._unit
        st = ctx.st
        g = ops.pool_bwd(ctx.y.shape, ctx.pooled, ctx.arg, as_cl(dout), *ctx.pool, relu=True)
        dy = unit.bn_backward(g, ctx.y, st)
        unit.backward(ctx.xcl, None, dy, need_dx=False)
        _notify(unit.params())
        ctx.xcl = ctx.y = ctx.pooled = ctx.arg = None
        return (None, None) + param_grads(ctx, 2)


class FuseFn(torch.autograd.Function):

    @staticmethod
    def forward(ctx, x_s, x_f, mod, *params):
        record_params(ctx, params)
        unit = mod._unit
        x_s, x_f = as_cl(x_s), as_cl(x_f)
        yf, st = unit.forward(x_f, None, mod.training)
        N, Cs, T, H, W = x_s.shape
        Cf = yf.shape[1]
        assert tuple(yf.shape) == (N, Cf, T, H, W), "lateral connection does not match the Slow pathway shape"
        cat = getattr(x_s, "_sf_cat", None)
        if cat is not None and tuple(cat.shape) == (N, Cs + Cf, T, H, W) and cat.data_ptr() == x_s.data_ptr():
            pass
        else:
            cat = ops.cl_empty((N, Cs + Cf, T, H, W), x_s.device)
            ops.bn_act(x_s, out=cat[:, :Cs])
        ops.bn_act(yf, st.scale, st.shift, relu=True, out=cat[:, Cs:])
        if CAPTURE is not None:
            CAPTURE.append({"kind": "fuse", "mod": mod, "raw": [yf], "bn": [(st.scale, st.shift)]})
        ctx.mod, ctx.yf, ctx.st, ctx.Cs = mod, yf, st, Cs
        ctx.save_for_backward(x_f)
        return cat, x_f.view_as(x_f)

    @staticmethod
    @delivers_grads
    def backward(ctx, dcat, dxf):
        unit = ctx.mod._unit
        (x_f,) = ctx.saved_tensors
        dcat = as_cl(dcat)
        dyf = unit.bn_backward(dcat[:, ctx.Cs:], ctx.yf, ctx.st, relu_self=True)
        need_dx = ctx.needs_input_grad[1]
        dx_f = unit.backward(x_f, None, dyf, need_dx=need_dx, resid=as_cl(dxf) if dxf is not None else None)
        _notify(unit.params())
        ctx.yf = None
        dx_s = dcat[:, :ctx.Cs] if ctx.needs_input_grad[0] else None
        return (dx_s, dx_f, None) + param_grads(ctx, 3)


class ResBlockFn(torch.autograd.Function):

    @staticmethod
    def forward(ctx, x, mod, *params):
        record_params(ctx, params)
        ctx.prev_bn = getattr(x, "_sf_block_bn", None) if BN_FUSE_REDUCE else None
        x = as_cl(x)
        units, P = mod.branch2._chain, mod._proj
        tr = mod.training
        raw, bn, act, h = [], [], [], x
        for i, u in enumerate(units):
            h, st = u.forward(h, None, tr)
            raw.append(h)
            bn.append(st)
            if i + 1 < len(units):
                h = ops.bn_act(h, st.scale, st.shift, relu=True)
                act.append(h)
        yc, sc = raw[-1], bn[-1]
        out_view, cat = None, None
        extra = getattr(mod, "_cat_extra", 0)
        if extra and CAT_IN_PLACE:
            N_, C_, T_, H_, W_ = yc.shape
            cat = ops.cl_empty((N_, C_ + extra, T_, H_, W_), x.device)
            out_view = cat[:, :C_]
        if P is not None:
            y1, s1 = P.forward(x, None, tr)
            out, bits = ops.bn_act(yc, sc.scale, sc.shift, relu=True, resid=y1, rscale=s1.scale, rshift=s1.shift,
                                   want_mask=True, out=out_view)
        else:
            y1, s1 = None, None
            out, bits = ops.bn_act(yc, sc.scale, sc.shift, relu=True, resid=x, want_mask=True, out=out_view)
        if cat is not None:
            out._sf_cat = cat
        if CAPTURE is not None:
            CAPTURE.append({"kind": "resblock", "mod": mod, "raw": list(raw), "bn": [(b.scale, b.shift) for b in bn], "out": out})
        ctx.mod = mod
        ctx.raw = (raw, y1, act, bits)
        ctx.bn = (bn, s1)
        ctx.save_for_backward(x)
        if BN_FUSE_REDUCE and tr:
            out._sf_block_bn = {"bits": bits, "y0": yc, "sync": _sync_of(units[-1].bn) is not None}
        return out

    @staticmethod
    @delivers_grads
    def backward(ctx, dout):
        mod = ctx.mod
        units, P = mod.branch2._chain, mod._proj
        (x,) = ctx.saved_tensors
        raw, y1, act, bits = ctx.raw
        bn, s1 = ctx.bn
        last = len(units) - 1
        part_c = tagged_bn_part(dout, raw[last])
        dout = as_cl(dout)
        need_dx = ctx.needs_input_grad[0]
        cgeom = units[last].fused_c_geom(act[last - 1]) if last > 0 else None
        if cgeom is None:
            dy = units[last].bn_backward(dout, raw[last], bn[last], zmask=bits, part=part_c)
        if P is not None:
            dy1 = P.bn_backward(dout, y1, s1, zmask=bits)
        for i in range(last, 0, -1):
            part = None
            if i == last and cgeom is not None:
                inner = (raw[i - 1], bn[i - 1]) if BN_FUSE_REDUCE and _sync_of(units[i - 1].bn) is None else None
                d_in, part = units[i].fused_c_backward(cgeom, act[i - 1], dout, raw[i], bn[i], bits, part=part_c, bn_fuse=inner)
            elif BN_FUSE_REDUCE and _sync_of(units[i - 1].bn) is None:
                d_in, part = units[i].backward(act[i - 1], None, dy, need_dx=True, bn_fuse=(raw[i - 1], bn[i - 1]))
            else:
                d_in = units[i].backward(act[i - 1], None, dy, need_dx=True)
            dy = units[i - 1].bn_backward(d_in, raw[i - 1], bn[i - 1], relu_self=True, part=part)
        prev = ctx.prev_bn if need_dx else None
        if prev is not None and prev["sync"]:
            prev = None
        if P is not None:
            dx1 = P.backward(x, None, dy1, need_dx=need_dx)
            dx = units[0].backward(x, None, dy, need_dx=need_dx, resid=dx1, bn_fuse=prev)
        else:
            dx = units[0].backward(x, None, dy, need_dx=need_dx, resid=dout, resid_bits=bits, bn_fuse=prev)
        if prev is not None:
            dx, pc = dx
            if pc is not None:
                tag_bn_part(dx, prev["y0"], pc)
        _notify(mod._param_list)
        ctx.raw = ctx.bn = ctx.prev_bn = None
        return (dx, None) + param_grads(ctx, 2)


CUT_BACKWARD = False
_cut_bn_tags = {}


def retag_cut_grad(g):
    tag = _cut_bn_tags.pop(g.data_ptr(), None)
    if tag is not None and getattr(g, "_sf_bn_part", None) is None and tag[2] == g.data_ptr() and tag[3] == g._version:
        g._sf_bn_part = tag


def tag_bn_part(dx, y0, part):
    dx._sf_bn_part = (y0.data_ptr(), part, dx.data_ptr(), dx._version)
    if CUT_BACKWARD:
        _cut_bn_tags[dx.data_ptr()] = dx._sf_bn_part


def tagged_bn_part(dout, y0):
    tag = getattr(dout, "_sf_bn_part", None)
    if tag is None or tag[0] != y0.data_ptr() or tag[2] != dout.data_ptr() or tag[3] != dout._version:
        return None
    return tag[1]


class ConvBNActFn(torch.autograd.Function):

    @staticmethod
    def forward(ctx, x, unit, relu, training, *params):
        record_params(ctx, params)
        x = as_cl(x)
        y, st = unit.forward(x, None, training)
        out = ops.bn_act(y, st.scale, st.shift, relu=relu)
        if CAPTURE is not None:
            CAPTURE.append({"kind": "convbnact", "mod": None, "raw": [y], "bn": [(st.scale, st.shift)], "out": out})
        ctx.unit, ctx.relu, ctx.y, ctx.st = unit, relu, y, st
        ctx.save_for_backward(x)
        return out

    @staticmethod
    @delivers_grads
    def backward(ctx, dout):
        unit = ctx.unit
        (x,) = ctx.saved_tensors
        dy = unit.bn_backward(as_cl(dout), ctx.y, ctx.st, relu_self=ctx.relu)
        dx = unit.backward(x, None, dy, need_dx=ctx.needs_input_grad[0])
        _notify(unit.params())
        ctx.y = None
        return (dx, None, None, None) + param_grads(ctx, 4)
```

slowfast_amd/lib.py:

```python
import ctypes
import os
from ctypes import POINTER, Structure, c_char_p, c_float, c_int, c_int32, c_int64, c_void_p

_HERE = os.path.dirname(os.path.abspath(__file__))
ABI_VERSION = 32
ACT_MODE = os.environ.get("SF_ACT_DTYPE", "fp16").lower()
if ACT_MODE not in ("fp16", "bf16"):
    raise ValueError(f"SF_ACT_DTYPE={ACT_MODE!r}: expected fp16 or bf16")
DEFAULT_LIBRARY = os.path.join(_HERE, "libsfamd.so" if ACT_MODE == "fp16" else "libsfamd_bf16.so")


def act_dtype():
    import torch
    return torch.float16 if ACT_MODE == "fp16" else torch.bfloat16


def act_eps():
    return 2.0 ** -11 if ACT_MODE == "fp16" else 2.0 ** -8


class ConvDesc(Structure):

    _fields_ = [(n, c_int32) for n in (
        "N", "Ci", "Ti", "Hi", "Wi", "Co", "To", "Ho", "Wo", "kT", "kH", "kW", "sT", "sH", "sW",
        "pT", "pH", "pW", "dT", "dH", "dW", "Cw", "ldx", "ldy", "Cow")]


class PrepItem(Structure):

    _fields_ = [("w", c_void_p), ("wf", c_void_p), ("wd", c_void_p)] + [(n, c_int32) for n in (
        "Co", "Cow", "Cw", "Cp", "taps", "ldf", "ldd", "pad")]


class DwDesc(Structure):

    _fields_ = [(n, c_int32) for n in (
        "N", "C", "Cw", "cls", "Ti", "Hi", "Wi", "To", "Ho", "Wo", "kT", "kH", "kW", "sT", "sH", "sW",
        "pT", "pH", "pW", "ldx", "ldy", "Cwreal")]


class Rows32(Structure):

    _fields_ = [("in_", c_void_p), ("out", c_void_p), ("ld", c_int32), ("period", c_int32)]


class ColFinItem(Structure):

    _fields_ = [("part", c_void_p), ("nblk", c_int32), ("C", c_int32), ("fold", c_int32), ("out0", c_void_p),
                ("out1", c_void_p), ("scale", c_float), ("accumulate", c_int32), ("row_stride", c_int32)]


class AttnDesc(Structure):

    _fields_ = [(n, c_int32) for n in (
        "B", "heads", "D", "cls", "Nq", "qT", "qH", "qW", "Nk", "kT", "kH", "kW", "rows_h", "rows_w", "rows_t")]


_P = c_void_p
_F = c_void_p
_SIGNATURES = {
    "sf_abi_version": (c_int, []),
    "sf_backend": (c_char_p, []),
    "sf_act_dtype": (c_int, []),
    "sf_last_error": (c_char_p, []),
    "sf_build_id": (c_char_p, []),
    "sf_conv_weight_ld": (c_int, [POINTER(ConvDesc), POINTER(c_int32), POINTER(c_int32)]),
    "sf_prep_weights": (c_int, [POINTER(ConvDesc), _F, _P, _P, _P]),
    "sf_prep_item_fill": (c_int, [POINTER(ConvDesc), _F, _P, _P, POINTER(PrepItem)]),
    "sf_prep_item_blocks": (c_int64, [POINTER(PrepItem)]),
    "sf_prep_weights_batch": (c_int, [_P, _P, _P, c_int32, _P]),
    "sf_conv_fwd_mtiles": (c_int, [POINTER(ConvDesc)]),
    "sf_conv_fwd": (c_int, [POINTER(ConvDesc), _P, _P, _F, _F, c_int, _F, _P, _F, _P]),
    "sf_conv_fwd_fused": (c_int, [POINTER(ConvDesc), _P, _P, _F, _P, c_int32, c_int, _P, _P]),
    "sf_conv_dgrad": (c_int, [POINTER(ConvDesc), _P, _P, _P, c_int32, _P, _P, _P]),
    "sf_conv_dgrad_bn": (c_int, [POINTER(ConvDesc), _P, _P, _P, c_int32, _P, _P, _P, _P, _P, _P, c_int32, _P, c_int32,
                                 POINTER(c_int32), _P]),
    "sf_conv_wgrad_workspace": (c_int64, [POINTER(ConvDesc)]),
    "sf_conv_wgrad_rowtab_bytes": (c_int64, [POINTER(ConvDesc)]),
    "sf_conv_wgrad_rowtab": (c_int, [POINTER(ConvDesc), _P, _P]),
    "sf_conv_wgrad": (c_int, [POINTER(ConvDesc), _P, _F, _F, c_int, _P, _F, c_float, c_int, _P, c_int64, _P, _P]),
    "sf_conv_c_bwd_plan": (c_int, [POINTER(ConvDesc), c_int, c_int, POINTER(c_int32), POINTER(c_int64)]),
    "sf_conv_c_bwd": (c_int, [POINTER(ConvDesc), _P, c_int32, _P, _P, c_int32, _F, _P, _P, _F, _F, _P, c_int32, _F, c_int32,
                              POINTER(c_int32), _P, c_int32, _F, c_float, c_int, _P, c_int64, _P]),
    "sf_bn_finalize": (c_int, [_F, c_int32, c_int32, c_int32, c_float, _F, _F, _F, _F, c_float, c_float, _F, _F, _F, _F, _P]),
    "sf_bn_act": (c_int, [c_int64, c_int32, _P, c_int32, _F, _F, _P, c_int32, _F, _F, c_int, _P, c_int32, _P, _P]),
    "sf_bn_bwd_blocks": (c_int, [c_int64, c_int32]),
    "sf_flat_blocks": (c_int, [c_int64]),
    "sf_flat_sumsq": (c_int, [_F, c_int64, _F, _P]),
    "sf_step_control": (c_int, [_F, c_int32, _F, c_float, c_float, c_int, c_float, c_float, c_int32, _P]),
    "sf_flat_sgd": (c_int, [_F, _F, _F, _P, _P, _P, c_int32, _F, _P, _P, c_int32, c_float, c_float, c_float, c_int, _P]),
    "sf_flat_adamw": (c_int, [_F, _F, _F, _F, _P, _P, _P, c_int32, _F, _P, _P, c_int32, c_float, c_float, c_float, c_float, _P]),
    "sf_flat_sgd_tab": (c_int, [_F, _F, _F, _P, _P, _P, c_int32, _F, _F, _F, c_float, c_float, c_float, c_int, _P]),
    "sf_flat_adamw_tab": (c_int, [_F, _F, _F, _F, _P, _P, _P, c_int32, _F, _F, _F, c_float, c_float, c_float, c_float, _P]),
    "sf_flat_lars_trust": (c_int, [_F, _F, _P, _P, _P, c_int32, _P, c_int32, _F, _F, _P, _F, c_float, c_float, c_float, _P]),
    "sf_bn_bwd_reduce": (c_int, [c_int64, c_int32, _P, c_int32, _P, c_int32, _P, c_int32, _F, _F, c_int, _F, _P]),
    "sf_bn_bwd_finalize": (c_int, [_F, c_int32, c_int32, c_int32, c_float, _F, _F, _F, c_float, _F, _F, c_int, _F, _P]),
    "sf_bn_bwd_apply": (c_int, [c_int64, c_int32, _P, c_int32, _P, c_int32, _P, c_int32, _F, _F, c_int, _F, _P,
                                c_int32, _P, c_int32, _P]),
    "sf_pool_fwd": (c_int, [c_int32] * 11 + [_P, c_int32, _F, _F, c_int, _P, c_int32, _P, c_int32, _P]),
    "sf_pool_bwd": (c_int, [c_int32] * 11 + [_P, c_int32, _P, c_int, _P, c_int32, _P, c_int32, c_int32, _P]),
    "sf_pool3d_fwd": (c_int, [c_int32] * 8 + [_P, c_int32, _P, c_int32, _P, _P]),
    "sf_pool3d_bwd": (c_int, [c_int32] * 8 + [_P, _P, c_int32, _P, c_int32, _P]),
    "sf_ncthw_to_cl": (c_int, [_F, c_int32, c_int32, c_int64, c_int32, _P, _P]),
    "sf_cl_to_ncthw": (c_int, [_P, c_int32, c_int32, c_int32, c_int64, _F, _P]),
    "sf_bgemm": (c_int, [c_int64, c_int32, c_int32, _P, c_int32, _P, c_int32, _F, _P, c_int32, _P, c_int32, c_int32,
                         c_int32] + [c_int64] * 8 + [c_int32, c_float, _P]),
    "sf_bgemm_tn": (c_int, [c_int64, c_int32, c_int32, _P, c_int32, _P, c_int32, _P, c_int32, c_float, c_int32, c_int32]
                    + [c_int64] * 6 + [_P]),
    "sf_layernorm_fwd": (c_int, [c_int64, c_int32, _P, c_int32, _F, _F, c_float, _P, c_int32, _F, _F, _P]),
    "sf_gemm_rows32": (c_int, [c_int64, c_int32, c_int32, _P, c_int32, _P, c_int32, _F, _P, c_int32, _P, c_int32,
                               POINTER(Rows32), _P]),
    "sf_layernorm_fwd_rows32": (c_int, [c_int64, c_int32, _P, c_int32, _F, _F, c_float, _P, c_int32, _F, _F,
                                        POINTER(Rows32), _P]),
    "sf_layernorm_bwd_blocks": (c_int, [c_int64, c_int32]),
    "sf_layernorm_bwd": (c_int, [c_int64, c_int32, _P, c_int32, _P, c_int32, _F, _F, _F, _P, c_int32, _P, c_int32, _F, _P]),
    "sf_layernorm_bwd_sums": (c_int, [c_int64, c_int32, _P, c_int32, _P, c_int32, _F, _F, _F, _P, c_int32, _P, c_int32, _F, _P]),
    "sf_colsum_blocks": (c_int, [c_int64, c_int32]),
    "sf_colsum": (c_int, [c_int64, c_int32, _P, c_int32, _F, _P]),
    "sf_colsum_finalize": (c_int, [_F, c_int32, c_int32, c_int32, _F, _F, c_float, c_int, _P]),
    "sf_colsum_finalize_batch": (c_int, [POINTER(ColFinItem), c_int32, _P]),
    "sf_rows_sum": (c_int, [_F, c_int32, c_int64, c_int64, c_int32, _F, c_float, c_int, _P]),
    "sf_gelu_fwd": (c_int, [c_int64, _P, _P, _P]),
    "sf_gelu_bwd": (c_int, [c_int64, _P, _P, _P, _P]),
    "sf_dwconv_fwd_blocks": (c_int, [POINTER(DwDesc)]),
    "sf_dwconv_fwd_sample_rows": (c_int, [POINTER(DwDesc)]),
    "sf_dwconv_pair_ok": (c_int, [POINTER(DwDesc)]),
    "sf_dwconv_fwd_pair": (c_int, [POINTER(DwDesc), _P, _P, _F, _F, _P, _P, _P]),
    "sf_dwconv_dgrad_pair": (c_int, [POINTER(DwDesc), _P, _P, _F, _F, _P, _P, _P]),
    "sf_dwconv_wgrad_pair": (c_int, [POINTER(DwDesc), _P, _P, _P, _P, _F, _F, c_float, c_int, c_int, _P, c_int64, _P]),
    "sf_dwconv_fwd": (c_int, [POINTER(DwDesc), _P, _F, _P, _F, _P]),
    "sf_dwconv_dgrad": (c_int, [POINTER(DwDesc), _P, _F, _P, _P]),
    "sf_dwconv_dgrad_sum_rows": (c_int, [POINTER(DwDesc)]),
    "sf_dwconv_dgrad_sums": (c_int, [POINTER(DwDesc), _P, _F, _P, _F, _P]),
    "sf_dwconv_wgrad_workspace": (c_int64, [POINTER(DwDesc)]),
    "sf_dwconv_wgrad": (c_int, [POINTER(DwDesc), _P, _P, _F, c_float, c_int, _P, c_int64, _P]),
    "sf_relpos_gather": (c_int, [POINTER(AttnDesc), _P, c_int32, _P, _P, _P, _F, _P]),
    "sf_relpos_scatter": (c_int, [POINTER(AttnDesc), _F, _P, _P, _P, _P, c_int32, _P]),
    "sf_relpos_pack": (c_int, [_F, _F, _F, c_int32, c_int32, c_int32, c_int32, c_int32, _P, _P, _P]),
    "sf_relpos_unpack": (c_int, [_F, c_int32, c_int32, c_int32, c_int32, _F, _F, _F, c_int32, c_int32, c_int32, _P]),
    "sf_softmax_fwd": (c_int, [POINTER(AttnDesc), _P, c_int32, c_float, _F, _P]),
    "sf_softmax_bwd": (c_int, [POINTER(AttnDesc), _P, _P, c_int32, c_float, _F, _P]),
    "sf_attn_fwd": (c_int, [POINTER(AttnDesc), _P, c_int32, _P, _P, c_int32, c_float, _F, _P, c_int32, _P, c_int32, _F, _P]),
    "sf_attn_bwd_workspace": (c_int64, [POINTER(AttnDesc)]),
    "sf_attn_bwd": (c_int, [POINTER(AttnDesc), _P, c_int32, _P, _P, c_int32, c_float, _F, _P, c_int32, _P, _P, c_int32, _F,
                            _F, _P, c_int32, _P, _P, c_int32, _F, _P, c_int64, _P]),
    "sf_tmean_fwd": (c_int, [c_int32, c_int32, c_int64, c_int32, _P, c_int32, _F, _P]),
    "sf_tmean_bwd": (c_int, [c_int32, c_int32, c_int64, c_int32, _F, _P, c_int32, _P]),
    "sf_roi_align_max_fwd": (c_int, [c_int32, c_int32, c_int32, c_int32, c_int32, c_int32, c_float, c_int32, _F, _F, _F,
                                     c_int32, c_int32, _P, _P]),
    "sf_roi_align_max_bwd": (c_int, [c_int32, c_int32, c_int32, c_int32, c_int32, c_int32, c_float, c_int32, _F, _F,
                                     c_int32, c_int32, _P, _F, _P]),
    "sf_gemm_act": (c_int, [c_int64, c_int32, c_int32, _P, c_int32, _P, c_int32, _F, _P, c_int32, c_int32, _P, c_int32, _P]),
    "sf_gemm_act_colsum": (c_int, [c_int64, c_int32, c_int32, _P, c_int32, _P, c_int32, _F, _P, c_int32, c_int32, _P, c_int32, _P, c_int32, POINTER(c_int32), _P]),
    "sf_pack_clip_u8": (c_int, [_P, c_int32, c_int32, c_int32, c_int32, _P, c_int32, c_float, c_float, c_float, c_float,
                                c_float, c_float, c_int32, _P, _P]),
    "sf_mix_clip_f32": (c_int, [_F, _F, c_int32, c_int32, c_int32, c_int32, c_int32, c_int32, c_float, c_float, c_int32, c_int32,
                                c_int32, c_int32, _P]),
    "sf_pack_clip_u8_mix": (c_int, [_P, c_int32, c_int32, c_int32, c_int32, _P, c_int32, c_float, c_float, c_float, c_float,
                                    c_float, c_float, c_int32, _P, c_int32, c_float, c_float, c_int32, c_int32, c_int32, c_int32,
                                    _P]),
    "sf_mix_targets": (c_int, [_P, c_int32, c_int32, c_float, c_float, c_float, c_float, _F, _P]),
    "sf_erase_clip_f32": (c_int, [_F, _F, c_int32, c_int32, c_int32, c_int32, c_int32, c_int32, _P, _P, c_int32, c_int32, _P]),
    "sf_pack_clip_u8_aug": (c_int, [_P, c_int32, c_int32, c_int32, c_int32, _P, c_int32, c_float, c_float, c_float, c_float,
                                    c_float, c_float, c_int32, _P, c_int32, _P, _P, c_int32, c_int32, c_int32, c_float, c_float,
                                    c_int32, c_int32, c_int32, c_int32, _P]),
    "sf_sample_clip_u8": (c_int, [_P, c_int32, c_int32, c_int32, c_int32, _P, _P, c_int32, c_float, c_float, c_float, c_float,
                                  c_float, c_float, _F, _P]),
    "sf_pack_clip_u8_sample": (c_int, [_P, c_int32, c_int32, c_int32, c_int32, _P, c_int32, c_float, c_float, c_float, c_float,
                                       c_float, c_float, c_int32, _P, _P, _P, c_int32, c_int32, _P, _P, c_int32, c_int32,
                                       c_int32, c_float, c_float, c_int32, c_int32, c_int32, c_int32, _P]),
    "sf_color_chunks": (c_int, [c_int64]),
    "sf_color_sum_depth": (c_int, []),
    "sf_color_frame_means_f32": (c_int, [_F, c_int32, c_int32, c_int64, _P, _P, _F, _F, _P]),
    "sf_color_clip_f32": (c_int, [_F, c_int32, c_int32, c_int64, _P, _P, _F, c_float, c_float, c_float, c_float, c_float,
                                  c_float, c_int32, _P]),
    "sf_randaug_chunk": (c_int, []),
    "sf_randaug_hist_u8": (c_int, [_P, c_int32, c_int32, c_int32, c_int32, _P, _P, _P, _P]),
    "sf_randaug_layer_u8": (c_int, [_P, _P, c_int32, c_int32, c_int32, c_int32, _P, _P, _P, _P, _P]),
    "sf_hog_targets_f32": (c_int, [_F, c_int32, c_int32, c_int32, c_int32, c_int32, c_int32, _F, _P]),
    "sf_mask_tokens_fwd": (c_int, [_P, c_int32, c_int32, c_int32, c_int32, c_int32, c_int32, c_int32, _P, c_int32, c_int32,
                                   c_int32, _F, _F, _P]),
    "sf_mask_tokens_bwd_blocks": (c_int, [c_int32, c_int32]),
    "sf_mask_tokens_bwd": (c_int, [_P, c_int32, _P, c_int32, c_int32, c_int32, c_int32, c_int32, c_int32, c_int32, _P, c_int32,
                                   c_int32, c_int32, _F, _F, _P]),
    "sf_token_keep_fwd": (c_int, [_P, c_int32, _P, c_int32, c_int32, c_int32, c_int32, c_int32, c_int32, _P, _P]),
    "sf_token_keep_bwd": (c_int, [_P, c_int32, _P, c_int32, c_int32, c_int32, c_int32, c_int32, c_int32, _P, _P]),
    "sf_token_restore_fwd": (c_int, [_P, c_int32, _P, c_int32, c_int32, c_int32, c_int32, c_int32, c_int32, _P, _F, _F, _P]),
    "sf_token_restore_bwd_blocks": (c_int, [c_int32, c_int32]),
    "sf_token_restore_bwd": (c_int, [_P, c_int32, _P, c_int32, c_int32, c_int32, c_int32, c_int32, c_int32, _P, _F, _F, _P]),
    "sf_pixel_targets_f32": (c_int, [_F, c_int32, c_int32, c_int32, c_int32, c_int32, c_int32, c_int32, c_int32, _F, _P]),
    "sf_row_scale_add": (c_int, [_P, c_int32, _P, c_int64, _P, c_int32, _P, c_int32, c_int64, c_int32, _P]),
    "sf_row_scale_add_rows32": (c_int, [_P, c_int32, _P, c_int64, _P, c_int32, _P, c_int32, c_int64, c_int32,
                                        POINTER(Rows32), _P]),
    "sf_transpose_heads": (c_int, [_P, c_int32, _P, c_int32, c_int32, c_int32, c_int32, c_int32, _P]),
    "sf_sample_chunks": (c_int, [c_int64, c_int32]),
    "sf_sample_mean": (c_int, [c_int32, c_int64, c_int32, _P, c_int32, _F, _F, c_int, _F, _F, _P]),
    "sf_se_gate_fwd": (c_int, [c_int32, c_int32, c_int32, c_int32, _F, _F, _F, _F, _F, _F, _F, _P]),
    "sf_gate_act_fwd": (c_int, [c_int32, c_int64, c_int32, _P, c_int32, _F, _F, _F, c_int, _P, c_int32, _P]),
    "sf_gate_grad": (c_int, [c_int32, c_int64, c_int32, _P, c_int32, _F, _F, _P, c_int32, _F, c_int, _F, _F, _P]),
    "sf_se_gate_bwd": (c_int, [c_int32, c_int32, c_int32, c_int32, _F, _F, _F, _F, _F, _F, _F, _F, _P]),
    "sf_outer_sum": (c_int, [_F, c_int32, _F, c_int32, c_int32, c_int32, c_int32, _F, c_float, c_int, _P]),
    "sf_gate_act_bwd": (c_int, [c_int32, c_int64, c_int32, _P, c_int32, _F, _F, _F, c_int, _P, c_int32, _F, _P, c_int32, _P]),
    "sf_gate_bwd_sums": (c_int, [c_int32, c_int64, c_int32, _P, c_int32, _F, _F, _P, c_int32, _F, c_int, _P, c_int32, _F, _F, _P]),
    "sf_bn_bwd_apply_sample": (c_int, [c_int64, c_int32, _P, c_int32, _P, c_int32, _F, _F, c_int64, _P, c_int32, _P]),
    "sf_gate_act_bwd_bn_rows": (c_int, [c_int32, c_int64, c_int32]),
    "sf_gate_act_bwd_bn": (c_int, [c_int32, c_int64, c_int32, _P, c_int32, _F, _F, _F, c_int, _P, c_int32, _F, _P, c_int32, _F, _P]),
}
EXPORTED_SYMBOLS = tuple(_SIGNATURES)


class SfError(RuntimeError):
    pass


class SfLibrary:
    def __init__(self, path):
        if not os.path.exists(path):
            raise SfError(
                f"native library not found: {path}. Build it with `python -m slowfast_amd.build_ext` "
                "(hipcc --offload-arch=gfx950); slowfast_amd has no CPU/PyTorch fallback.")
        self.path = path
        self.cdll = ctypes.CDLL(path)
        for name, (res, args) in _SIGNATURES.items():
            fn = getattr(self.cdll, name)
            fn.restype = res
            fn.argtypes = args
        ver = self.cdll.sf_abi_version()
        if ver != ABI_VERSION:
            raise SfError(f"{path}: ABI version {ver}, expected {ABI_VERSION}")
        self.backend = self.cdll.sf_backend().decode()
        self.build_id = self.cdll.sf_build_id().decode()
        from . import build_ext
        if build_ext.sources_present():
            want = build_ext.source_id(sim=self.backend == "hostsim")
            if self.build_id != want and os.environ.get("SF_ALLOW_STALE_LIBRARY", "0") == "0":
                raise SfError(f"{path} was built from other sources (build id {self.build_id}, sources {want}): rebuild with "
# ... 39 lines not shown
```

slowfast_amd/ops.py:

```python
from ctypes import byref, c_int32, c_int64

import torch

from . import lib as _sflib

from .lib import ConvDesc, SfError, get_lib

_f16 = _sflib.act_dtype()


def _triple(v):
    return tuple(v) if isinstance(v, (tuple, list)) else (v, v, v)


def _stream(t):
    if t.is_cuda:
        return torch.cuda.current_stream(t.device).cuda_stream
    if get_lib().backend != "hostsim":
        raise SfError("slowfast_amd kernels need CUDA/HIP tensors (got a CPU tensor and the gfx950 library)")
    return None


def _ptr(t):
    return None if t is None else t.data_ptr()
# ... 201 lines not shown
                       work=geom.work(reads_x=1 + int(resid is not None), reads_y=1, writes_x=1))
        return dx, (part[:nrows.value] if nrows.value > 0 else None)
    ldy = cl_ld(dy)
    dx = cl_empty(geom.in_shape, dy.device) if out is None else out
    ldx = cl_ld(dx)
    ldr = cl_ld(resid) if resid is not None else 0
    if resid_bits is not None:
        assert resid is not None and resid_bits.dtype == torch.uint8 and resid_bits.numel() == rows(resid) * (geom.Ci // 8)
    get_lib().call("sf_conv_dgrad", byref(geom.desc(ldx, ldy)), dy.data_ptr(), wd.data_ptr(), _ptr(resid), ldr,
                   _ptr(resid_bits), dx.data_ptr(), _stream(dy),
                   work=geom.work(reads_x=int(resid is not None), reads_y=1, writes_x=1))
    return dx


_workspaces = {}
_retired_workspaces = []


def _workspace(device, nbytes):
    sid = torch.cuda.current_stream(device).cuda_stream if device.type == "cuda" else 0
    k = (device, sid)
    ws = _workspaces.get(k)
    if ws is None or ws.numel() < nbytes:
        if ws is not None:
            _retired_workspaces.append(ws)
        ws = torch.empty(max(int(nbytes * 1.25), 1 << 20), dtype=torch.uint8, device=device)
        _workspaces[k] = ws
    return ws


def conv_wgrad(x, dy, geom, dw, in_affine=None, out_scale=1.0, zero_first=True):
    assert tuple(x.shape) == geom.in_shape and tuple(dy.shape) == geom.out_shape
    assert dw.dtype == torch.float32 and dw.is_contiguous() and dw.numel() == geom.Cow * geom.Cw * geom.taps
    sc, sh, relu = _affine(in_affine)
    lib = get_lib()
    d = geom.desc(cl_ld(x), cl_ld(dy))
    if geom.ws_bytes is None:
        geom.ws_bytes = lib.call("sf_conv_wgrad_workspace", byref(d))
    ws = _workspace(x.device, geom.ws_bytes)
    lib.call("sf_conv_wgrad", byref(d), x.data_ptr(), _ptr(sc), _ptr(sh), relu,
                   dy.data_ptr(), dw.data_ptr(), float(out_scale), int(zero_first), ws.data_ptr(), ws.numel(),
                   _ptr(_wgrad_rowtab(geom, d, x.device)) if sc is None else None, _stream(x),
                   work=geom.work(reads_x=1, reads_y=1))
    return dw


_rowtabs = {}


def _capturing(device):
    return device.type == "cuda" and torch.cuda.is_current_stream_capturing()


def _wgrad_rowtab(geom, d, device):
    nbytes = getattr(geom, "_rowtab_bytes", None)
    if nbytes is None:
        nbytes = geom._rowtab_bytes = get_lib().call("sf_conv_wgrad_rowtab_bytes", byref(d))
    if nbytes <= 0:
        return None
    key = (device, 0, geom.N, geom.Ti, geom.Hi, geom.Wi, geom.To, geom.Ho, geom.Wo, geom.k, geom.s, geom.p, geom.d)
    if key not in _rowtabs:
        tab = torch.empty(nbytes, dtype=torch.uint8, device=device)
        get_lib().call("sf_conv_wgrad_rowtab", byref(d), tab.data_ptr(), _stream(tab))
        if _capturing(device):
            return tab
        if device.type == "cuda":
            torch.cuda.current_stream(device).synchronize()
        _rowtabs[key] = tab
    return _rowtabs[key]


def bn_finalize(part, count, gamma, beta, running_mean, running_var, momentum, eps, training=True, C=None):
    Creal = gamma.numel()
    C = C or (part.shape[2] if part is not None else Creal)
    dev = gamma.device
    scale, shift, mean, rstd = (torch.empty(C, dtype=torch.float32, device=dev) for _ in range(4))
    nblk = part.shape[0] if training else 0
    get_lib().call("sf_bn_finalize", _ptr(part) if training else None, nblk, C, Creal, float(count), gamma.data_ptr(),
                   beta.data_ptr(), _ptr(running_mean), _ptr(running_var), float(momentum), float(eps),
                   scale.data_ptr(), shift.data_ptr(), mean.data_ptr(), rstd.data_ptr(), _stream(gamma))
    return scale, shift, mean, rstd


def bn_act(y, scale=None, shift=None, relu=False, resid=None, rscale=None, rshift=None, out=None, want_mask=False):
    ldy = cl_ld(y)
    N, C, T, H, W = y.shape
    out = cl_empty(y.shape, y.device) if out is None else out
    assert tuple(out.shape) == tuple(y.shape)
    mask = torch.empty((rows(y), C // 8), dtype=torch.uint8, device=y.device) if want_mask else None
    get_lib().call("sf_bn_act", rows(y), C, y.data_ptr(), ldy, _ptr(scale), _ptr(shift), _ptr(resid),
                   cl_ld(resid) if resid is not None else 0, _ptr(rscale), _ptr(rshift), int(bool(relu)),
                   out.data_ptr(), cl_ld(out), _ptr(mask), _stream(y),
                   work=dict(bytes=2.0 * y.numel() * (2 + int(resid is not None) + (1 / 16 if want_mask else 0))))
    return (out, mask) if want_mask else out


def bn_bwd(dz, y, gamma, mean, rstd, dgamma, dbeta, zmask=None, relu_affine=None, inv_loss_scale=1.0,
           accumulate=False, want_g=False, out=None, sync=None, part=None, sample_add=None, coef_only=False):
    lib = get_lib()
    N, C, T, H, W = y.shape
    M = rows(y)
    s = _stream(y)
    fused_part = part
    if fused_part is None:
        nblk = lib.call("sf_bn_bwd_blocks", M, C)
        part = torch.empty((nblk, 2, C), dtype=torch.float32, device=y.device)
    else:
        assert part.dtype == torch.float32 and part.is_contiguous() and tuple(part.shape[1:]) == (2, C)
        nblk = part.shape[0]
    sc, sh = (relu_affine if relu_affine is not None else (None, None))
    relu_self = int(relu_affine is not None)
    bits = zmask is not None and zmask.dtype == torch.uint8
    if bits:
        assert zmask.numel() == M * (C // 8) and zmask.is_contiguous()
    mcost = 0.0 if zmask is None else (1 / 16 if bits else 1.0)
    lddz, ldy, ldm = cl_ld(dz), cl_ld(y), (0 if bits or zmask is None else cl_ld(zmask))
    if fused_part is None:
        lib.call("sf_bn_bwd_reduce", M, C, dz.data_ptr(), lddz, _ptr(zmask), ldm, y.data_ptr(), ldy, _ptr(sc), _ptr(sh),
                 relu_self, part.data_ptr(), s, work=dict(bytes=2.0 * y.numel() * (2 + mcost)))
    coef = torch.empty((3, C), dtype=torch.float32, device=y.device)
    if sync is None:
        lib.call("sf_bn_bwd_finalize", part.data_ptr(), nblk, C, gamma.numel(), float(M), gamma.data_ptr(), mean.data_ptr(),
                 rstd.data_ptr(), float(inv_loss_scale), dgamma.data_ptr(), dbeta.data_ptr(), int(accumulate),
                 coef.data_ptr(), s)
    else:
        import torch.distributed as dist
        group, gsize = sync
        tot = part.sum(0, keepdim=True)
        loc = tot.clone()
        lib.call("sf_bn_bwd_finalize", loc.data_ptr(), 1, C, gamma.numel(), float(M), gamma.data_ptr(), mean.data_ptr(),
                 rstd.data_ptr(), float(inv_loss_scale), dgamma.data_ptr(), dbeta.data_ptr(), int(accumulate),
                 coef.data_ptr(), s)
        dist.all_reduce(tot, group=group)
        scratch = torch.empty((2, gamma.numel()), dtype=torch.float32, device=y.device)
        lib.call("sf_bn_bwd_finalize", tot.data_ptr(), 1, C, gamma.numel(), float(M) * gsize, gamma.data_ptr(),
                 mean.data_ptr(), rstd.data_ptr(), float(inv_loss_scale), scratch[0].data_ptr(), scratch[1].data_ptr(), 0,
                 coef.data_ptr(), s)
    if coef_only:
        return coef
    dy = cl_empty(y.shape, y.device) if out is None else out
    if sample_add is not None:
        assert fused_part is not None and zmask is None and relu_affine is None and not want_g
        assert sample_add.dtype == torch.float32 and sample_add.is_contiguous() and tuple(sample_add.shape) == (N, C)
        lib.call("sf_bn_bwd_apply_sample", M, C, dz.data_ptr(), lddz, y.data_ptr(), ldy, coef.data_ptr(), sample_add.data_ptr(),
                 M // N, dy.data_ptr(), cl_ld(dy), s, work=dict(bytes=2.0 * y.numel() * 3))
        return dy
    g = cl_empty(y.shape, y.device) if want_g else None
    lib.call("sf_bn_bwd_apply", M, C, dz.data_ptr(), lddz, _ptr(zmask), ldm, y.data_ptr(), ldy, _ptr(sc), _ptr(sh),
             relu_self, coef.data_ptr(), dy.data_ptr(), cl_ld(dy), _ptr(g), cl_ld(g) if g is not None else 0, s,
             work=dict(bytes=2.0 * y.numel() * (3 + mcost + int(want_g))))
    return (dy, g) if want_g else dy


def bn_bwd_coef(dz, y, gamma, mean, rstd, dgamma, dbeta, zmask=None, inv_loss_scale=1.0, accumulate=False, part=None):
    return bn_bwd(dz, y, gamma, mean, rstd, dgamma, dbeta, zmask=zmask, inv_loss_scale=inv_loss_scale, accumulate=accumulate,
                  part=part, coef_only=True)


def conv_c_bwd_plan(geom, in_affine=False, mask_bits=True):
    tile_rows, ws = c_int32(0), c_int64(0)
    ok = get_lib().call("sf_conv_c_bwd_plan", byref(geom.desc(geom.Ci, geom.Co)), int(bool(in_affine)), int(bool(mask_bits)),
                        byref(tile_rows), byref(ws))
    return (tile_rows.value, ws.value) if ok == 1 else None


def conv_c_bwd(dz, bits, yc, coef, act, wd, geom, dw, bn=None, out_scale=1.0, zero_first=True, out=None):
    plan = conv_c_bwd_plan(geom)
    assert plan is not None, "conv_c_bwd: the planner rejects this geometry"
    tile_rows, ws_bytes = plan
    assert tuple(act.shape) == geom.in_shape and tuple(dz.shape) == geom.out_shape and tuple(yc.shape) == geom.out_shape
    assert dw.dtype == torch.float32 and dw.is_contiguous() and dw.numel() == geom.Cow * geom.Cw * geom.taps
    M = rows(yc)
    assert bits.dtype == torch.uint8 and bits.is_contiguous() and bits.numel() == M * (geom.Co // 8)
    assert coef.dtype == torch.float32 and coef.is_contiguous() and tuple(coef.shape) == (3, geom.Co)
    d_in = cl_empty(geom.in_shape, dz.device) if out is None else out
    assert tuple(d_in.shape) == geom.in_shape
    part, cap, nrows = None, 0, c_int32(0)
    y0 = sc = sh = None
    if bn is not None:
        y0, sc, sh = bn
        assert tuple(y0.shape) == geom.in_shape
        cap = (M + tile_rows - 1) // tile_rows
        part = torch.empty((cap, 2, geom.Ci), dtype=torch.float32, device=dz.device)
    ws = _workspace(dz.device, ws_bytes)
    W = 2.0 * M * geom.Co
    get_lib().call("sf_conv_c_bwd", byref(geom.desc(cl_ld(act), geom.Co)), dz.data_ptr(), cl_ld(dz), bits.data_ptr(), yc.data_ptr(),
                   cl_ld(yc), coef.data_ptr(), act.data_ptr(), wd.data_ptr(), _ptr(sc), _ptr(sh), _ptr(y0),
                   cl_ld(y0) if y0 is not None else 0, _ptr(part), cap, byref(nrows), d_in.data_ptr(), cl_ld(d_in), dw.data_ptr(),
                   float(out_scale), int(zero_first), ws.data_ptr(), ws.numel(), _stream(dz),
                   work=dict(flops=4.0 * M * geom.Co * geom.Cw,
                             bytes=W * (2 + 1 / 16) + 2.0 * M * geom.Ci * (2 + int(bn is not None))))
    return d_in, (part[:nrows.value] if part is not None and nrows.value > 0 else None)


def _pool_args(y, kernel, stride, padding):
    N, C, T, H, W = y.shape
    (kH, kW), (sH, sW), (pH, pW) = kernel, stride, padding
    return (N, T, H, W, C, kH, kW, sH, sW, pH, pW), ((H + 2 * pH - kH) // sH + 1, (W + 2 * pW - kW) // sW + 1)


def pool_fwd(y, kernel, stride, padding, affine=None, want_argmax=True):
    args, (Ho, Wo) = _pool_args(y, kernel, stride, padding)
    N, C, T, H, W = y.shape
    out = cl_empty((N, C, T, Ho, Wo), y.device)
    arg = torch.empty((N, T, Ho, Wo, C), dtype=torch.uint8, device=y.device) if want_argmax else None
    sc, sh, relu = _affine(affine)
    get_lib().call("sf_pool_fwd", *args, y.data_ptr(), cl_ld(y), _ptr(sc), _ptr(sh), relu, out.data_ptr(),
                   cl_ld(out), _ptr(arg), 0, _stream(y), work=dict(bytes=2.0 * (y.numel() + out.numel())))
    return out, arg


def pool_bwd(in_shape, pooled, argmax, dout, kernel, stride, padding, relu=True):
    N, C, T, H, W = in_shape
    (kH, kW), (sH, sW), (pH, pW) = kernel, stride, padding
    assert tuple(dout.shape) == tuple(pooled.shape)
    g = cl_empty(in_shape, dout.device)
    get_lib().call("sf_pool_bwd", N, T, H, W, C, kH, kW, sH, sW, pH, pW, pooled.data_ptr(), cl_ld(pooled),
                   argmax.data_ptr(), int(bool(relu)), dout.data_ptr(), cl_ld(dout), g.data_ptr(), cl_ld(g), 0,
                   _stream(dout), work=dict(bytes=2.0 * (g.numel() + 2.5 * dout.numel())))
    return g
```

Baseline: 903.8 clips/s.

## Recompute thin 1x1x1 conv outputs instead of storing them for BN

Adds a family of thin-conv kernels that recompute the output of cheap 1x1x1 convolutions from the input activation and weights. They do this in a stats pass, a fused BN-affine/residual/ReLU tail pass and a backward BN-reduce pass, so the conv output y_c is never written to or read from HBM. The fused conv_c backward gains a template variant that rebuilds y_c in LDS from the activation tile rather than loading it. This trades HBM traffic and memory footprint for extra MFMA work plus additional kernel launches and passes over the activations. The path is on by default through a test hook and a row-count gate.

```diff
diff --git a/include/sfamd.h b/include/sfamd.h
--- a/include/sfamd.h
+++ b/include/sfamd.h
@@ -6,7 +6,7 @@
 extern "C" {
 #endif
 
-#define SF_ABI_VERSION 32
+#define SF_ABI_VERSION 33
 typedef void* sf_stream_t;
 
 typedef struct sf_conv_desc {
@@ -65,6 +65,15 @@
                   const void* bn_y, int32_t bn_ldy, float* bn_part, int32_t bn_part_rows, int32_t* bn_rows, void* d_in,
                   int32_t ld_in, float* dw, float out_scale, int zero_first, void* workspace, int64_t workspace_bytes,
                   sf_stream_t stream);
+int sf_conv_c_thin_plan(const sf_conv_desc* d, int has_bias, int sync_stats, int batch_stats);
+int sf_conv_c_rows(const sf_conv_desc* d);
+int sf_conv_c_bwd_reduce_rows(const sf_conv_desc* d, int epilogue_order);
+int sf_conv_c_stats(const sf_conv_desc* d, const void* act, const void* wd, float* part, int32_t part_rows, sf_stream_t stream);
+int sf_conv_c_tail(const sf_conv_desc* d, const void* act, const void* wd, const float* scale, const float* shift,
+                   const void* resid, int32_t ldr, const float* rscale, const float* rshift, int relu, void* out, int32_t ldo,
+                   void* mask_out, sf_stream_t stream);
+int sf_conv_c_bwd_reduce(const sf_conv_desc* d, const void* act, const void* wd, const void* dz, int32_t lddz,
+                         const void* mask_bits, int epilogue_order, float* part, int32_t part_rows, sf_stream_t stream);
 
 int sf_bn_finalize(float* part, int32_t nblk, int32_t C, int32_t Creal, float count, const float* gamma, const float* beta,
                    float* running_mean, float* running_var, float momentum, float eps, float* scale, float* shift,
diff --git a/slowfast_amd/csrc/sf_api.hip b/slowfast_amd/csrc/sf_api.hip
--- a/slowfast_amd/csrc/sf_api.hip
+++ b/slowfast_amd/csrc/sf_api.hip
@@ -5,6 +5,7 @@
 #include "sf_igemm2.h"
 #include "sf_wgrad2.h"
 #include "sf_cbwd.h"
+#include "sf_cthin.h"
 #include "sf_pool.h"
 #include "sf_dwconv.h"
 #include "sf_dwsweep.h"
@@ -940,7 +941,9 @@
                              int32_t* bn_rows, void* d_in, int32_t ld_in, float* dw, float out_scale, int zero_first,
                              void* workspace, int64_t workspace_bytes, sf_stream_t stream) {
     if (check_desc(d)) return -1;
-    REQUIRE(dz && mask_bits && yc && coef && act && wd && d_in && dw && workspace, "sf_conv_c_bwd: null pointer");
+    REQUIRE(dz && mask_bits && coef && act && wd && d_in && dw && workspace, "sf_conv_c_bwd: null pointer");
+    const bool rc = yc == nullptr;
+    if (rc) ldyc = d->Co;
     const CbwdPlan w = plan_cbwd(d, false, true);
     REQUIRE(w.ok, "sf_conv_c_bwd: this geometry keeps sf_bn_bwd_apply + sf_conv_wgrad + sf_conv_dgrad_bn (sf_conv_c_bwd_plan == 0)");
     REQUIRE(lddz >= d->Co && lddz % 8 == 0 && ldyc >= d->Co && ldyc % 8 == 0 && ld_in >= d->Ci && ld_in % 8 == 0,
@@ -981,11 +984,76 @@
         REQUIRE(wgs <= SF_CBWD_MAX_WGS, "sf_conv_c_bwd: %d splits", wgs);
     }
     hipStream_t s = (hipStream_t)stream;
-    SF_CBWD_FOR_SHAPE(w.cip, w.cop, hipLaunchKernelGGL((sf_cbwd_kernel<CIP_, COP_>), dim3(wgs), dim3(SF_THREADS), 0, s, p));
+    if (rc) SF_CBWD_FOR_SHAPE(w.cip, w.cop, hipLaunchKernelGGL((sf_cbwd_kernel<CIP_, COP_, true>), dim3(wgs), dim3(SF_THREADS), 0, s, p));
+    else SF_CBWD_FOR_SHAPE(w.cip, w.cop, hipLaunchKernelGGL((sf_cbwd_kernel<CIP_, COP_>), dim3(wgs), dim3(SF_THREADS), 0, s, p));
     if (check_launch("conv_c_bwd")) return -1;
     if (bn_rows) *bn_rows = fuse ? ntiles : 0;
     launch_wgrad_reduce(d, (const float*)workspace, wgs, w.cop, w.cip, false, dw, out_scale, zero_first, s);
     return check_launch("conv_c_bwd_reduce");
+}
+
+static bool plan_cthin_rows_ok(const sf_conv_desc* d) {
+    const int64_t M = (int64_t)d->N * d->Ti * d->Hi * d->Wi;
+    return !(d->Ci > 32 && d->Co > 128) || M >= test_hook("SF_CTHIN_MINROWS", 131072);
+}
+static bool plan_cthin(const sf_conv_desc* d, bool has_bias, bool sync_stats, bool batch_stats) {
+    if (test_hook("SF_CTHIN", 1) == 0) return false;
+    if (has_bias || sync_stats || !batch_stats || !plan_cthin_rows_ok(d)) return false;
+    return plan_cbwd(d, false, true).ok;
+}
+extern "C" int sf_conv_c_thin_plan(const sf_conv_desc* d, int has_bias, int sync_stats, int batch_stats) {
+    if (check_desc(d)) return -1;
+    return plan_cthin(d, has_bias != 0, sync_stats != 0, batch_stats != 0) ? 1 : 0;
+}
+
+static int cthin_common(const char* who, const sf_conv_desc* d, const void* act, const void* wd, CthinParams& p, CbwdPlan& w, int& wgs) {
+    if (check_desc(d)) return -1;
+    REQUIRE(act && wd, "%s: null pointer", who);
+    w = plan_cbwd(d, false, true);
+    REQUIRE(w.ok, "%s: not a thin 1x1x1 convolution (sf_conv_c_bwd_plan == 0)", who);
+    REQUIRE(d->ldx >= d->Ci && d->ldx % 8 == 0 && (((uintptr_t)act | (uintptr_t)wd) & 15) == 0, "%s: bad act pitch / alignment", who);
+    const int64_t M = (int64_t)d->N * d->Ti * d->Hi * d->Wi;
+    REQUIRE(M > 0 && M < (1ll << 31) - 256, "%s: bad row count", who);
+    int32_t ldf, ldd;
+    sf_conv_weight_ld(d, &ldf, &ldd);
+    memset(&p, 0, sizeof(p));
+    p.M = (int)M; p.Ci = d->Ci; p.Co = d->Co; p.act = (const f16*)act; p.ldact = d->ldx; p.wd = (const f16*)wd; p.ldw = ldd;
+    p.tiles128 = cdiv(M, 128);
+    const int forced = test_hook("SF_CTHIN_WGS", 0);
+    wgs = forced > 0 ? forced : 2048;
+    if (wgs > p.tiles128) wgs = p.tiles128;
+    return 0;
+}
+#define SF_CTHIN_LAUNCH(mode) \
+    SF_CBWD_FOR_SHAPE(w.cip, w.cop, hipLaunchKernelGGL((sf_cthin_kernel<CIP_, COP_, mode>), dim3(wgs), dim3(SF_THREADS), 0, (hipStream_t)stream, p))
+
+extern "C" int sf_conv_c_rows(const sf_conv_desc* d) {
+    if (check_desc(d)) return -1;
+    return cdiv((int64_t)d->N * d->Ti * d->Hi * d->Wi, 128);
+}
+extern "C" int sf_conv_c_stats(const sf_conv_desc* d, const void* act, const void* wd, float* part, int32_t part_rows,
+                               sf_stream_t stream) {
+    CthinParams p; CbwdPlan w; int wgs;
+    if (cthin_common("sf_conv_c_stats", d, act, wd, p, w, wgs)) return -1;
+    REQUIRE(part && part_rows >= p.tiles128, "sf_conv_c_stats: the table needs ceil(positions / 128) rows of [2][Co] floats");
+    p.part = part;
+    SF_CTHIN_LAUNCH(CTHIN_STATS);
+    return check_launch("conv_c_stats");
+}
+
+extern "C" int sf_conv_c_tail(const sf_conv_desc* d, const void* act, const void* wd, const float* scale, const float* shift,
+                              const void* resid, int32_t ldr, const float* rscale, const float* rshift, int relu, void* out,
+                              int32_t ldo, void* mask_out, sf_stream_t stream) {
+    CthinParams p; CbwdPlan w; int wgs;
+    if (cthin_common("sf_conv_c_tail", d, act, wd, p, w, wgs)) return -1;
+    REQUIRE(out && ldo >= d->Co && ldo % 8 == 0 && ((uintptr_t)out & 15) == 0, "sf_conv_c_tail: bad out pitch / alignment");
+    REQUIRE((scale == nullptr) == (shift == nullptr) && (rscale == nullptr) == (rshift == nullptr), "sf_conv_c_tail: scale / shift come together");
+    REQUIRE(!resid || (ldr >= d->Co && ldr % 8 == 0 && ((uintptr_t)resid & 15) == 0), "sf_conv_c_tail: bad residual pitch / alignment");
+    REQUIRE(resid || !rscale, "sf_conv_c_tail: a residual affine without a residual");
+    p.scale = scale; p.shift = shift; p.resid = (const f16*)resid; p.ldr = ldr; p.rscale = rscale; p.rshift = rshift; p.relu = relu;
+    p.out = (f16*)out; p.ldo = ldo; p.mask_out = (uint8_t*)mask_out;
+    SF_CTHIN_LAUNCH(CTHIN_TAIL);
+    return check_launch("conv_c_tail");
 }
 
 static RowTile make_rowtile(int64_t M, int C, int max_blocks, dim3& grid) {
@@ -1068,6 +1136,35 @@
     p.y = (const f16*)y; p.ldy = ldy; p.scale = scale; p.shift = shift; p.relu_self = relu_self; p.part = part;
     hipLaunchKernelGGL(sf_bn_bwd_reduce_kernel, grid, dim3(SF_THREADS), 0, (hipStream_t)stream, p);
     return check_launch("bn_bwd_reduce");
+}
+
+static int cthin_reduce_blocks() {
+    const int forced = test_hook("SF_CTHIN_BLOCKS", 0);
+    return forced > 0 ? forced : kBwdBlocks;
+}
+extern "C" int sf_conv_c_bwd_reduce_rows(const sf_conv_desc* d, int epilogue_order) {
+    if (check_desc(d)) return -1;
+    const int64_t M = (int64_t)d->N * d->Ti * d->Hi * d->Wi;
+    if (epilogue_order) return cdiv(M, 128);
+    dim3 grid;
+    make_rowtile(M, d->Co, cthin_reduce_blocks(), grid);
+    return (int)grid.x;
+}
+extern "C" int sf_conv_c_bwd_reduce(const sf_conv_desc* d, const void* act, const void* wd, const void* dz, int32_t lddz,
+                                    const void* mask_bits, int epilogue_order, float* part, int32_t part_rows, sf_stream_t stream) {
+    CthinParams p; CbwdPlan w; int wgs;
+    if (cthin_common("sf_conv_c_bwd_reduce", d, act, wd, p, w, wgs)) return -1;
+    REQUIRE(dz && mask_bits && lddz >= d->Co && lddz % 8 == 0 && ((uintptr_t)dz & 15) == 0, "sf_conv_c_bwd_reduce: bad dz / mask");
+    if (!epilogue_order) {
+        dim3 grid;
+        const RowTile rt = make_rowtile(p.M, d->Co, cthin_reduce_blocks(), grid);
+        p.rpb = rt.rows_per_block; wgs = (int)grid.x;
+    }
+    const int rows = epilogue_order ? p.tiles128 : wgs;
+    REQUIRE(part && part_rows >= rows, "sf_conv_c_bwd_reduce: the table needs sf_conv_c_bwd_reduce_rows rows of [2][Co] floats");
+    p.dz = (const f16*)dz; p.lddz = lddz; p.bits = (const uint8_t*)mask_bits; p.part = part;
+    SF_CTHIN_LAUNCH(CTHIN_REDUCE);
+    return check_launch("conv_c_bwd_reduce_rc");
 }
 
 extern "C" int sf_bn_bwd_finalize(float* part, int32_t nblk, int32_t C, int32_t Creal, float count, const float* gamma,
diff --git a/slowfast_amd/csrc/sf_cbwd.h b/slowfast_amd/csrc/sf_cbwd.h
--- a/slowfast_amd/csrc/sf_cbwd.h
+++ b/slowfast_amd/csrc/sf_cbwd.h
@@ -2,6 +2,7 @@
 #include "sf_bn.h"
 #include "sf_common.h"
 #include "sf_igemm.h"
+#include "sf_cthin.h"
 
 struct CbwdParams {
     int M, Ci, Co;
@@ -44,7 +45,7 @@
     static_assert(SF_THREADS % ACH == 0 && 64 % ACH == 0, "a thread keeps one d_in column group");
 };
 
-template <int CIP, int COP>
+template <int CIP, int COP, bool RC = false>
 __global__ __launch_bounds__(SF_THREADS, (CbwdCfg<CIP, COP>::OCC)) void sf_cbwd_kernel(CbwdParams p) {
     using K = CbwdCfg<CIP, COP>;
     constexpr int R = K::R, LDY = K::LDY, NJ = K::NJ, TI = K::TI, TC = K::TC;
@@ -104,7 +105,7 @@
             int m = m0 + srow + u * K::RPP;
             if (m > p.M - 1) m = p.M - 1;
             dzr[u] = ld16(p.dz + (int64_t)m * p.lddz + scgc * 8);
-            ycr[u] = ld16(p.yc + (int64_t)m * p.ldyc + scgc * 8);
+            if constexpr (!RC) ycr[u] = ld16(p.yc + (int64_t)m * p.ldyc + scgc * 8);
             mbr[u] = p.bits[(int64_t)m * (p.Co >> 3) + scgc];
         }
     };
@@ -123,7 +124,8 @@
             if (q < K::NACT) {
                 const int c = q * 64 + lane;
                 const int m = m0 + c / K::ACH, cc = c % K::ACH;
-                const f16* g = (m >= r0 && m < r1 && cc * 8 < p.Ci) ? p.act + (int64_t)m * p.ldact + cc * 8 : zline;
+                const bool mine = RC ? m < p.M : (m >= r0 && m < r1);
+                const f16* g = (mine && cc * 8 < p.Ci) ? p.act + (int64_t)m * p.ldact + cc * 8 : zline;
                 SF_GLOBAL_LOAD_LDS16_ASM(g, ActL + q * 512);
             }
         }
@@ -151,6 +153,16 @@
         const bool more = q + 1 < nq;
         SF_WAIT_VMEM();
         __syncthreads();
+        if constexpr (RC) {
+            cthin_tile_store<CIP, COP, R>(ActL, WdL, DyL, wave, lane);
+            __syncthreads();
+            if (m0 < r0 || m0 + R > r1) {
+                for (int c = tid; c < R * K::ACH; c += SF_THREADS) {
+                    const int m = m0 + c / K::ACH;
+                    if (m < r0 || m >= r1) st16(ActL + c * 8, zero8());
+                }
+            }
+        }
         {
             float k1[8], k2[8], k3[8];
 #pragma unroll
@@ -159,7 +171,9 @@
             for (int u = 0; u < K::NCH; ++u) {
                 const int row = srow + u * K::RPP;
                 const uint32_t b = mbr[u];
-                const f16x8 yv = ycr[u];
+                f16x8 yv;
+                if constexpr (RC) yv = ld16(DyL + row * LDY + scg * 8);
+                else yv = ycr[u];
                 float g[8];
 #pragma unroll
                 for (int e = 0; e < 8; ++e) g[e] = (float)dzr[u][e];
diff --git a/slowfast_amd/csrc/sf_cthin.h b/slowfast_amd/csrc/sf_cthin.h
--- /dev/null
+++ b/slowfast_amd/csrc/sf_cthin.h
@@ -0,0 +1,346 @@
+#pragma once
+#include "sf_bn.h"
+#include "sf_common.h"
+#include "sf_igemm.h"
+#include <type_traits>
+
+template <int CIP, int COP, int R>
+struct CthinTile {
+    static constexpr int LDY = COP + 8;
+    static constexpr bool ROWS = R == 128;
+    static constexpr int TI = ROWS ? 2 : 4;
+    static constexpr int KS = CIP <= 32 ? 1 : 2;
+    static constexpr int NJ = COP / 16;
+    static constexpr int NJW = ROWS ? NJ : NJ / 4;
+    static constexpr int JC = NJW < 4 ? NJW : (ROWS ? 4 : 2);
+    static_assert((R == 128 || R == 64) && NJW >= 1 && NJW % JC == 0, "tile shape");
+    __device__ static __forceinline__ int row0(int wave) { return ROWS ? wave * 32 : 0; }
+    __device__ static __forceinline__ int col0(int wave) { return ROWS ? 0 : wave * NJW; }
+};
+
+template <int CIP, int COP, int R, class Sink>
+__device__ __forceinline__ void cthin_tile(const f16* ActL, const f16* WdL, int wave, int lane, Sink&& sink) {
+    using T = CthinTile<CIP, COP, R>;
+    const int pl = lane & 15, g4 = lane >> 4;
+    const int rowbase = T::row0(wave), j0 = T::col0(wave);
+#pragma unroll
+    for (int jc = 0; jc < T::NJW; jc += T::JC) {
+        f32x4 acc[T::TI][T::JC];
+#pragma unroll
+        for (int i = 0; i < T::TI; ++i)
+#pragma unroll
+            for (int j = 0; j < T::JC; ++j) acc[i][j] = (f32x4){0.f, 0.f, 0.f, 0.f};
+#pragma unroll
+        for (int ks = 0; ks < T::KS; ++ks) {
+            const int k0 = ks * 32 + 8 * g4;
+            const bool kok = k0 < CIP;
+            const int kc = kok ? k0 : 0;
+            f16x8 af[T::TI];
+#pragma unroll
+            for (int i = 0; i < T::TI; ++i) {
+                af[i] = zero8();
+                if (kok) af[i] = ld16(ActL + (rowbase + i * 16 + pl) * CIP + k0);
+            }
+#pragma unroll
+            for (int j = 0; j < T::JC; ++j) {
+                f16x8 bf;
+#pragma unroll
+                for (int h = 0; h < 2; ++h) {
+                    const f16x4 v = as_f16x4(SF_LDS_TR16(WdL + (kc + 4 * h + (pl >> 2)) * T::LDY + (j0 + jc + j) * 16 + 4 * (pl & 3)));
+                    bf[4 * h + 0] = v[0]; bf[4 * h + 1] = v[1]; bf[4 * h + 2] = v[2]; bf[4 * h + 3] = v[3];
+                }
+                if (!kok) bf = zero8();
+#pragma unroll
+                for (int i = 0; i < T::TI; ++i) acc[i][j] = SF_MFMA16(af[i], bf, acc[i][j]);
+            }
+        }
+        sink(jc, acc);
+    }
+}
+
+template <int CIP, int COP, int R>
+__device__ __forceinline__ void cthin_tile_store(const f16* ActL, const f16* WdL, f16* YL, int wave, int lane) {
+    using T = CthinTile<CIP, COP, R>;
+    const int pl = lane & 15, g4 = lane >> 4;
+    const int rowbase = T::row0(wave), j0 = T::col0(wave);
+    cthin_tile<CIP, COP, R>(ActL, WdL, wave, lane, [&](int jc, f32x4 (&acc)[T::TI][T::JC]) {
+#pragma unroll
+        for (int i = 0; i < T::TI; ++i)
+#pragma unroll
+            for (int j = 0; j < T::JC; ++j)
+#pragma unroll
+                for (int r = 0; r < 4; ++r) YL[(rowbase + i * 16 + 4 * g4 + r) * T::LDY + (j0 + jc + j) * 16 + pl] = (f16)acc[i][j][r];
+    });
+}
+
+enum { CTHIN_STATS = 0, CTHIN_TAIL = 1, CTHIN_REDUCE = 2 };
+
+struct CthinParams {
+    int M, Ci, Co;
+    const f16* act; int ldact;
+    const f16* wd; int ldw;
+    int tiles128;
+    float* part;
+    int rpb;
+    const float* scale; const float* shift;
+    const f16* resid; int ldr;
+    const float* rscale; const float* rshift;
+    int relu;
+    f16* out; int ldo;
+    uint8_t* mask_out;
+    const f16* dz; int lddz;
+    const uint8_t* bits;
+};
+
+template <int CIP, int COP, int MODE>
+struct CthinCfg {
+    static constexpr int R = COP >= 128 ? 64 : 128;
+    static constexpr int NSUB = 128 / R;
+    static constexpr int LDY = COP + 8;
+    static constexpr int CGO = COP / 8, RPP = SF_THREADS / CGO, NCH = R / RPP;
+    static constexpr int ACH = CIP / 8, NACT = R * ACH / 64;
+    static constexpr int Y_ELEMS = MODE == CTHIN_STATS ? 0 : R * LDY;
+    static constexpr int ACT_ELEMS = R * CIP, WD_ELEMS = CIP * LDY;
+    static constexpr int NBUF = MODE == CTHIN_STATS ? 2 : 1;
+    static constexpr int RED_ELEMS = MODE == CTHIN_STATS ? 4 * 2 * COP * 2 : 0;
+    static constexpr int CGE = CGO < 16 ? CGO : 16, NHE = CGO / CGE;
+    static_assert(MODE != CTHIN_REDUCE || (4 * CGO * 24 * 2 <= Y_ELEMS && 4 * CGO * 17 * 2 <= Y_ELEMS), "the reduction scratch fits the y_c tile");
+    static constexpr int LDS_ELEMS = Y_ELEMS + NBUF * ACT_ELEMS + WD_ELEMS + RED_ELEMS;
+    static constexpr int OCC = LDS_ELEMS * 2 * 4 <= 160 * 1024 ? 4 : 2;
+    static_assert(R % RPP == 0 && NACT >= 1 && (R * ACH) % 64 == 0 && 64 % CGO == 0, "tile shape");
+};
+
+template <int CIP, int COP, int MODE>
+__global__ __launch_bounds__(SF_THREADS, (CthinCfg<CIP, COP, MODE>::OCC)) void sf_cthin_kernel(CthinParams p) {
+    using K = CthinCfg<CIP, COP, MODE>;
+    using T = CthinTile<CIP, COP, K::R>;
+    constexpr int R = K::R, LDY = K::LDY;
+    __shared__ __attribute__((aligned(16))) f16 smem[K::LDS_ELEMS];
+    f16* const YL = smem;
+    f16* const ActL0 = smem + K::Y_ELEMS;
+    f16* const WdL = ActL0 + K::NBUF * K::ACT_ELEMS;
+    float* const red = reinterpret_cast<float*>(MODE == CTHIN_REDUCE ? YL : WdL + K::WD_ELEMS);
+
+    const int tid = threadIdx.x;
+    const int lane = tid & 63, wave = __builtin_amdgcn_readfirstlane(tid >> 6);
+    const int G = (int)gridDim.x;
+    const f16* const zline = reinterpret_cast<const f16*>(sf_zero_line);
+
+    for (int q = tid; q < CIP * K::CGO; q += SF_THREADS) {
+        const int ci = q / K::CGO, cg = q % K::CGO;
+        f16x8 v = zero8();
+        if (ci < p.Ci && cg * 8 < p.Co) v = ld16(p.wd + (int64_t)ci * p.ldw + cg * 8);
+        st16(WdL + ci * LDY + cg * 8, v);
+    }
+
+    const int scg = tid % K::CGO, srow = tid / K::CGO;
+    const bool scol_ok = scg * 8 < p.Co;
+    const int scgc = scol_ok ? scg : 0;
+
+    const int T0 = (int)blockIdx.x;
+    const bool blocks = MODE == CTHIN_REDUCE && p.rpb > 0;
+    const int rb0 = blocks ? T0 * p.rpb : 0;
+    const int rend = blocks && rb0 + p.rpb < p.M ? rb0 + p.rpb : p.M;
+    const int nq = blocks ? (rend - rb0 + R - 1) / R : T0 < p.tiles128 ? ((p.tiles128 - 1 - T0) / G + 1) * K::NSUB : 0;
+    auto tile_T = [&](int q) { return T0 + (q / K::NSUB) * G; };
+    auto tile_m0 = [&](int q) { return blocks ? rb0 + q * R : tile_T(q) * 128 + (q % K::NSUB) * R; };
+    auto issue_act = [&](int m0, f16* ActL) {
+#pragma unroll
+        for (int j = 0; j < (K::NACT + 3) / 4; ++j) {
+            const int q = wave + 4 * j;
+            if (q < K::NACT) {
+                const int c = q * 64 + lane;
+                const int m = m0 + c / K::ACH, cc = c % K::ACH;
+                const f16* g = (m < p.M && cc * 8 < p.Ci) ? p.act + (int64_t)m * p.ldact + cc * 8 : zline;
+                SF_GLOBAL_LOAD_LDS16_ASM(g, ActL + q * 512);
+            }
+        }
+    };
+
+    float sc[8], sh[8], rsc[8], rsh[8];
+#pragma unroll
+    for (int e = 0; e < 8; ++e) { sc[e] = 1.f; sh[e] = 0.f; rsc[e] = 1.f; rsh[e] = 0.f; }
+    if constexpr (MODE == CTHIN_TAIL) {
+        if (p.scale && scol_ok) { load8f(p.scale + scg * 8, sc); load8f(p.shift + scg * 8, sh); }
+        if (p.resid && p.rscale && scol_ok) { load8f(p.rscale + scg * 8, rsc); load8f(p.rshift + scg * 8, rsh); }
+    }
+    const bool ident = MODE == CTHIN_TAIL && !p.scale && !p.resid && !p.relu;
+    float ss[T::NJW], sq[T::NJW];
+    float sg[K::NHE][8], sgy[K::NHE][8];
+    const float one[8] = {1.f, 1.f, 1.f, 1.f, 1.f, 1.f, 1.f, 1.f}, zero[8] = {0.f, 0.f, 0.f, 0.f, 0.f, 0.f, 0.f, 0.f};
+#pragma unroll
+    for (int j = 0; j < T::NJW; ++j) { ss[j] = 0.f; sq[j] = 0.f; }
+#pragma unroll
+    for (int h = 0; h < K::NHE; ++h)
+#pragma unroll
+        for (int e = 0; e < 8; ++e) { sg[h][e] = 0.f; sgy[h][e] = 0.f; }
+    auto with_map = [&](auto&& f) {
+        if (K::NHE > 1 && !blocks) f(std::integral_constant<int, K::CGE>{}, std::integral_constant<int, K::NHE>{});
+        else f(std::integral_constant<int, K::CGO>{}, std::integral_constant<int, 1>{});
+    };
+
+    if (nq > 0) issue_act(tile_m0(0), ActL0);
+    for (int q = 0; q < nq; ++q) {
+        const int m0 = tile_m0(q);
+        const bool more = q + 1 < nq;
+        f16* const ActL = ActL0 + (K::NBUF == 2 ? (q & 1) * K::ACT_ELEMS : 0);
+        f16x8 opr[K::NCH];
+        uint32_t mbr[K::NCH];
+        if constexpr (MODE != CTHIN_STATS) {
+#pragma unroll
+            for (int u = 0; u < K::NCH; ++u) {
+                int m = m0 + srow + u * K::RPP;
+                if (m > p.M - 1) m = p.M - 1;
+                opr[u] = zero8();
+                mbr[u] = 0u;
+                if constexpr (MODE == CTHIN_TAIL) {
+                    if (p.resid) opr[u] = ld16(p.resid + (int64_t)m * p.ldr + scgc * 8);
+                }
+            }
+        }
+        if constexpr (MODE == CTHIN_REDUCE) {
+            with_map([&](auto cgc, auto nhc) {
+                constexpr int CG = decltype(cgc)::value, NH = decltype(nhc)::value, NU = R * CG / SF_THREADS;
+#pragma unroll
+                for (int u = 0; u < NU; ++u)
+#pragma unroll
+                    for (int h = 0; h < NH; ++h) {
+                        int m = m0 + (tid + u * SF_THREADS) / CG;
+                        if (m > p.M - 1) m = p.M - 1;
+                        int cg = tid % CG + h * CG;
+                        if (cg * 8 >= p.Co) cg = 0;
+                        opr[u * NH + h] = ld16(p.dz + (int64_t)m * p.lddz + cg * 8);
+                        mbr[u * NH + h] = p.bits[(int64_t)m * (p.Co >> 3) + cg];
+                    }
+            });
+        }
+        SF_WAIT_VMEM();
+        __syncthreads();
+        if constexpr (MODE == CTHIN_STATS) {
+            if (more) issue_act(tile_m0(q + 1), ActL0 + ((q + 1) & 1) * K::ACT_ELEMS);
+            cthin_tile<CIP, COP, R>(ActL, WdL, wave, lane, [&](int jc, f32x4 (&acc)[T::TI][T::JC]) {
+#pragma unroll
+                for (int j = 0; j < T::JC; ++j) {
+                    float s = 0.f, v2 = 0.f;
+#pragma unroll
+                    for (int i = 0; i < T::TI; ++i)
+#pragma unroll
+                        for (int r = 0; r < 4; ++r) {
+                            const float v = acc[i][j][r];
+                            s += v;
+                            v2 += v * v;
+                        }
+                    ss[jc + j] += wave_sum_over_row_groups(s);
+                    sq[jc + j] += wave_sum_over_row_groups(v2);
+                }
+            });
+        } else {
+            cthin_tile_store<CIP, COP, R>(ActL, WdL, YL, wave, lane);
+        }
+        if constexpr (MODE != CTHIN_STATS) {
+            __syncthreads();
+            if (more) issue_act(tile_m0(q + 1), ActL);
+        }
+        if constexpr (MODE == CTHIN_TAIL) {
+#pragma unroll
+            for (int u = 0; u < K::NCH; ++u) {
+                const int row = srow + u * K::RPP, m = m0 + row;
+                if (!(scol_ok && m < p.M)) continue;
+                const f16x8 v = ld16(YL + row * LDY + scg * 8);
+                f16x8 o;
+                uint32_t bits = 0;
+                if (ident) o = v;
+                else {
+                    float x[8];
+#pragma unroll
+                    for (int e = 0; e < 8; ++e) x[e] = (float)v[e] * sc[e] + sh[e];
+                    if (p.resid) {
+                        const f16x8 rv = opr[u];
+#pragma unroll
+                        for (int e = 0; e < 8; ++e) x[e] += (float)rv[e] * rsc[e] + rsh[e];
+                    }
+#pragma unroll
+                    for (int e = 0; e < 8; ++e) {
+                        float t = x[e];
+                        if (p.relu) t = t > 0.f ? t : 0.f;
+                        o[e] = (f16)t;
+                    }
+                }
+#pragma unroll
+                for (int e = 0; e < 8; ++e) bits |= (o[e] > (f16)0.f ? 1u : 0u) << e;
+                st16(p.out + (int64_t)m * p.ldo + scg * 8, o);
+                if (p.mask_out) p.mask_out[(int64_t)m * (p.Co >> 3) + scg] = (uint8_t)bits;
+            }
+        } else if constexpr (MODE == CTHIN_REDUCE) {
+            with_map([&](auto cgc, auto nhc) {
+                constexpr int CG = decltype(cgc)::value, NH = decltype(nhc)::value, NU = R * CG / SF_THREADS;
+#pragma unroll
+                for (int u = 0; u < NU; ++u)
+#pragma unroll
+                    for (int h = 0; h < NH; ++h) {
+                        const int row = (tid + u * SF_THREADS) / CG, m = m0 + row, cg = tid % CG + h * CG;
+                        if (!(cg * 8 < p.Co && m < rend)) continue;
+                        const f16x8 v = ld16(YL + row * LDY + cg * 8);
+                        bnb_accumulate(opr[u * NH + h], v, one, zero, sg[h], sgy[h], true, mbr[u * NH + h]);
+                    }
+            });
+        }
+        if (blocks ? more : q % K::NSUB != K::NSUB - 1) continue;
+        float* prow = p.part + (int64_t)(blocks ? T0 : tile_T(q)) * 2 * p.Co;
+        if constexpr (MODE == CTHIN_STATS) {
+            if constexpr (T::ROWS) {
+#pragma unroll
+                for (int j = 0; j < T::NJW; ++j) {
+                    if (lane < 16) { red[(wave * 2 + 0) * COP + j * 16 + lane] = ss[j]; red[(wave * 2 + 1) * COP + j * 16 + lane] = sq[j]; }
+                    ss[j] = 0.f; sq[j] = 0.f;
+                }
+                __syncthreads();
+                if (tid < COP && tid < p.Co) {
+                    float s = 0.f, v = 0.f;
+#pragma unroll
+                    for (int w = 0; w < 4; ++w) { s += red[(w * 2 + 0) * COP + tid]; v += red[(w * 2 + 1) * COP + tid]; }
+                    prow[tid] = s;
+                    prow[p.Co + tid] = v;
+                }
+            } else {
+#pragma unroll
+                for (int j = 0; j < T::NJW; ++j) {
+                    const int col = (T::col0(wave) + j) * 16 + lane;
+                    if (lane < 16 && col < p.Co) { prow[col] = ss[j]; prow[p.Co + col] = sq[j]; }
+                    ss[j] = 0.f; sq[j] = 0.f;
+                }
+            }
+        } else if constexpr (MODE == CTHIN_REDUCE) {
+            if (blocks) {
+                constexpr int TG = K::CGO;
+                float (*s_red)[17] = reinterpret_cast<float (*)[17]>(red);
+#pragma unroll
+                for (int e = 0; e < 8; ++e)
+                    for (int mask = TG; mask < SF_WAVE; mask <<= 1) {
+                        sg[0][e] += __shfl_xor(sg[0][e], mask);
+                        sgy[0][e] += __shfl_xor(sgy[0][e], mask);
+                    }
+                __syncthreads();
+                if (lane < TG) {
+#pragma unroll
+                    for (int e = 0; e < 8; ++e) { s_red[wave * TG + lane][e] = sg[0][e]; s_red[wave * TG + lane][8 + e] = sgy[0][e]; }
+                }
+                __syncthreads();
+                if (tid < TG && tid * 8 < p.Co) {
+#pragma unroll
+                    for (int e = 0; e < 8; ++e) {
+                        prow[tid * 8 + e] = (s_red[tid][e] + s_red[TG + tid][e]) + (s_red[2 * TG + tid][e] + s_red[3 * TG + tid][e]);
+                        prow[p.Co + tid * 8 + e] = (s_red[tid][8 + e] + s_red[TG + tid][8 + e]) + (s_red[2 * TG + tid][8 + e] + s_red[3 * TG + tid][8 + e]);
+                    }
+                }
+            } else {
+#pragma unroll
+                for (int h = 0; h < K::NHE; ++h) {
+                    bnb_reduce_store<4, K::CGE>(sg[h], sgy[h], red, prow, h * K::CGE * 8, p.Co);
+#pragma unroll
+                    for (int e = 0; e < 8; ++e) { sg[h][e] = 0.f; sgy[h][e] = 0.f; }
+                }
+            }
+        }
+    }
+}
diff --git a/slowfast_amd/engine.py b/slowfast_amd/engine.py
--- a/slowfast_amd/engine.py
+++ b/slowfast_amd/engine.py
@@ -398,13 +398,25 @@
         geom = self.geom(x.shape)
         return geom if ops.conv_c_bwd_plan(geom) is not None else None
 
-    def fused_c_backward(self, geom, x, dz, y, st, bits, part=None, bn_fuse=None):
+    def thin_c_geom(self, x, training):
+        if self.bn is None or not self.conv.weight.requires_grad:
+            return None
+        geom = self.geom(x.shape)
+        ok = ops.conv_c_thin_plan(geom, has_bias=self.conv.bias is not None, sync_stats=_sync_of(self.bn) is not None,
+                                  batch_stats=training or self.bn.running_mean is None)
+        return geom if ok else None
+
+    def thin_c_statistics(self, geom, x, training):
+        _, wd = self.weights(geom, fresh=True)
+        return wd, bn_statistics(self.bn, ops.conv_c_stats(x, wd, geom), geom.out_rows, geom.Co, training)
+
+    def fused_c_backward(self, geom, x, dz, y, st, bits, part=None, bn_fuse=None, epilogue_order=False):
         bn = self.bn
         dgamma, dbeta, accumulate = self._bn_grad_dest()
+        _, wd = self.weights(geom)
         coef = ops.bn_bwd_coef(dz, y, bn.weight, st.mean, st.rstd, dgamma, dbeta, zmask=bits, inv_loss_scale=1.0,
-                               accumulate=accumulate, part=part)
+                               accumulate=accumulate, part=part, thin=(x, wd, geom, epilogue_order))
         dw, zero_first = _grad_dest(self.conv.weight)
-        _, wd = self.weights(geom)
         fuse = None
         if bn_fuse is not None:
             y0, st0 = bn_fuse
@@ -611,7 +623,15 @@
         units, P = mod.branch2._chain, mod._proj
         tr = mod.training
         raw, bn, act, h = [], [], [], x
+        tgeom = twd = None
         for i, u in enumerate(units):
+            if i > 0 and i + 1 == len(units):
+                tgeom = u.thin_c_geom(h, tr)
+                if tgeom is not None:
+                    twd, st = u.thin_c_statistics(tgeom, h, tr)
+                    raw.append(None)
+                    bn.append(st)
+                    break
             h, st = u.forward(h, None, tr)
             raw.append(h)
             bn.append(st)
@@ -622,21 +642,25 @@
         out_view, cat = None, None
         extra = getattr(mod, "_cat_extra", 0)
         if extra and CAT_IN_PLACE:
-            N_, C_, T_, H_, W_ = yc.shape
+            N_, C_, T_, H_, W_ = yc.shape if tgeom is None else tgeom.out_shape
             cat = ops.cl_empty((N_, C_ + extra, T_, H_, W_), x.device)
             out_view = cat[:, :C_]
-        if P is not None:
-            y1, s1 = P.forward(x, None, tr)
-            out, bits = ops.bn_act(yc, sc.scale, sc.shift, relu=True, resid=y1, rscale=s1.scale, rshift=s1.shift,
-                                   want_mask=True, out=out_view)
+        y1, s1 = P.forward(x, None, tr) if P is not None else (None, None)
+        tail = dict(relu=True, want_mask=True, out=out_view)
+        tail.update(dict(resid=x) if P is None else dict(resid=y1, rscale=s1.scale, rshift=s1.shift))
+        if tgeom is not None:
+            out, bits = ops.conv_c_tail(h, twd, tgeom, sc.scale, sc.shift, **tail)
         else:
-            y1, s1 = None, None
-            out, bits = ops.bn_act(yc, sc.scale, sc.shift, relu=True, resid=x, want_mask=True, out=out_view)
+            out, bits = ops.bn_act(yc, sc.scale, sc.shift, **tail)
         if cat is not None:
             out._sf_cat = cat
         if CAPTURE is not None:
+            if tgeom is not None:
+                raw = raw[:-1] + [ops.conv_c_tail(h, twd, tgeom)]
             CAPTURE.append({"kind": "resblock", "mod": mod, "raw": list(raw), "bn": [(b.scale, b.shift) for b in bn], "out": out})
         ctx.mod = mod
+        if tgeom is not None:
+            raw = raw[:-1] + [None]
         ctx.raw = (raw, y1, act, bits)
         ctx.bn = (bn, s1)
         ctx.save_for_backward(x)
@@ -653,10 +677,15 @@
         raw, y1, act, bits = ctx.raw
         bn, s1 = ctx.bn
         last = len(units) - 1
-        part_c = tagged_bn_part(dout, raw[last])
+        thin_order = False
+        if raw[last] is not None:
+            part_c = tagged_bn_part(dout, raw[last])
+        else:
+            part_c, thin_order = None, tagged_bn_part(dout, bits) is THIN_EPILOGUE_ORDER
         dout = as_cl(dout)
         need_dx = ctx.needs_input_grad[0]
         cgeom = units[last].fused_c_geom(act[last - 1]) if last > 0 else None
+        assert cgeom is not None or raw[last] is not None, "a block whose y_c was never stored needs the fused conv c backward"
         if cgeom is None:
             dy = units[last].bn_backward(dout, raw[last], bn[last], zmask=bits, part=part_c)
         if P is not None:
@@ -665,7 +694,8 @@
             part = None
             if i == last and cgeom is not None:
                 inner = (raw[i - 1], bn[i - 1]) if BN_FUSE_REDUCE and _sync_of(units[i - 1].bn) is None else None
-                d_in, part = units[i].fused_c_backward(cgeom, act[i - 1], dout, raw[i], bn[i], bits, part=part_c, bn_fuse=inner)
+                d_in, part = units[i].fused_c_backward(cgeom, act[i - 1], dout, raw[i], bn[i], bits, part=part_c, bn_fuse=inner,
+                                                       epilogue_order=thin_order)
             elif BN_FUSE_REDUCE and _sync_of(units[i - 1].bn) is None:
                 d_in, part = units[i].backward(act[i - 1], None, dy, need_dx=True, bn_fuse=(raw[i - 1], bn[i - 1]))
             else:
@@ -674,15 +704,18 @@
         prev = ctx.prev_bn if need_dx else None
         if prev is not None and prev["sync"]:
             prev = None
+        fuse0 = prev if prev is not None and prev["y0"] is not None else None
         if P is not None:
             dx1 = P.backward(x, None, dy1, need_dx=need_dx)
-            dx = units[0].backward(x, None, dy, need_dx=need_dx, resid=dx1, bn_fuse=prev)
+            dx = units[0].backward(x, None, dy, need_dx=need_dx, resid=dx1, bn_fuse=fuse0)
         else:
-            dx = units[0].backward(x, None, dy, need_dx=need_dx, resid=dout, resid_bits=bits, bn_fuse=prev)
-        if prev is not None:
+            dx = units[0].backward(x, None, dy, need_dx=need_dx, resid=dout, resid_bits=bits, bn_fuse=fuse0)
+        if fuse0 is not None:
             dx, pc = dx
             if pc is not None:
                 tag_bn_part(dx, prev["y0"], pc)
+        elif prev is not None and tuple(units[0].conv.stride) == (1, 1, 1):
+            tag_bn_part(dx, prev["bits"], THIN_EPILOGUE_ORDER)
         _notify(mod._param_list)
         ctx.raw = ctx.bn = ctx.prev_bn = None
         return (dx, None) + param_grads(ctx, 2)
@@ -696,6 +729,9 @@
     tag = _cut_bn_tags.pop(g.data_ptr(), None)
     if tag is not None and getattr(g, "_sf_bn_part", None) is None and tag[2] == g.data_ptr() and tag[3] == g._version:
         g._sf_bn_part = tag
+
+
+THIN_EPILOGUE_ORDER = "thin block: the consumer's data-gradient epilogue would have taken the sums"
 
 
 def tag_bn_part(dx, y0, part):
diff --git a/slowfast_amd/lib.py b/slowfast_amd/lib.py
--- a/slowfast_amd/lib.py
+++ b/slowfast_amd/lib.py
@@ -3,7 +3,7 @@
 from ctypes import POINTER, Structure, c_char_p, c_float, c_int, c_int32, c_int64, c_void_p
 
 _HERE = os.path.dirname(os.path.abspath(__file__))
-ABI_VERSION = 32
+ABI_VERSION = 33
 ACT_MODE = os.environ.get("SF_ACT_DTYPE", "fp16").lower()
 if ACT_MODE not in ("fp16", "bf16"):
     raise ValueError(f"SF_ACT_DTYPE={ACT_MODE!r}: expected fp16 or bf16")
@@ -82,6 +82,12 @@
     "sf_conv_c_bwd_plan": (c_int, [POINTER(ConvDesc), c_int, c_int, POINTER(c_int32), POINTER(c_int64)]),
     "sf_conv_c_bwd": (c_int, [POINTER(ConvDesc), _P, c_int32, _P, _P, c_int32, _F, _P, _P, _F, _F, _P, c_int32, _F, c_int32,
                               POINTER(c_int32), _P, c_int32, _F, c_float, c_int, _P, c_int64, _P]),
+    "sf_conv_c_thin_plan": (c_int, [POINTER(ConvDesc), c_int, c_int, c_int]),
+    "sf_conv_c_rows": (c_int, [POINTER(ConvDesc)]),
+    "sf_conv_c_bwd_reduce_rows": (c_int, [POINTER(ConvDesc), c_int]),
+    "sf_conv_c_stats": (c_int, [POINTER(ConvDesc), _P, _P, _F, c_int32, _P]),
+    "sf_conv_c_tail": (c_int, [POINTER(ConvDesc), _P, _P, _F, _F, _P, c_int32, _F, _F, c_int, _P, c_int32, _P, _P]),
+    "sf_conv_c_bwd_reduce": (c_int, [POINTER(ConvDesc), _P, _P, _P, c_int32, _P, c_int, _F, c_int32, _P]),
     "sf_bn_finalize": (c_int, [_F, c_int32, c_int32, c_int32, c_float, _F, _F, _F, _F, c_float, c_float, _F, _F, _F, _F, _P]),
     "sf_bn_act": (c_int, [c_int64, c_int32, _P, c_int32, _F, _F, _P, c_int32, _F, _F, c_int, _P, c_int32, _P, _P]),
     "sf_bn_bwd_blocks": (c_int, [c_int64, c_int32]),
diff --git a/slowfast_amd/ops.py b/slowfast_amd/ops.py
--- a/slowfast_amd/ops.py
+++ b/slowfast_amd/ops.py
@@ -377,7 +377,25 @@
     return (dy, g) if want_g else dy
 
 
-def bn_bwd_coef(dz, y, gamma, mean, rstd, dgamma, dbeta, zmask=None, inv_loss_scale=1.0, accumulate=False, part=None):
+def bn_bwd_coef(dz, y, gamma, mean, rstd, dgamma, dbeta, zmask=None, inv_loss_scale=1.0, accumulate=False, part=None, thin=None):
+    if y is None:
+        act, wd, geom, order = thin
+        C, M = geom.Co, rows(act)
+        assert zmask is not None and zmask.dtype == torch.uint8 and zmask.is_contiguous() and zmask.numel() == M * (C // 8)
+        lib = get_lib()
+        if part is None:
+            d = geom.desc(cl_ld(act), C)
+            nblk = lib.call("sf_conv_c_bwd_reduce_rows", byref(d), int(bool(order)))
+            part = torch.empty((nblk, 2, C), dtype=torch.float32, device=dz.device)
+            lib.call("sf_conv_c_bwd_reduce", byref(d), act.data_ptr(), wd.data_ptr(), dz.data_ptr(), cl_ld(dz), zmask.data_ptr(),
+                     int(bool(order)), part.data_ptr(), nblk, _stream(dz),
+                     work=dict(flops=2.0 * M * C * geom.Cw, bytes=2.0 * M * (C * (1 + 1 / 16) + geom.Ci)))
+        assert part.dtype == torch.float32 and part.is_contiguous() and tuple(part.shape[1:]) == (2, C)
+        coef = torch.empty((3, C), dtype=torch.float32, device=dz.device)
+        lib.call("sf_bn_bwd_finalize", part.data_ptr(), part.shape[0], C, gamma.numel(), float(M), gamma.data_ptr(), mean.data_ptr(),
+                 rstd.data_ptr(), float(inv_loss_scale), dgamma.data_ptr(), dbeta.data_ptr(), int(accumulate), coef.data_ptr(),
+                 _stream(dz))
+        return coef
     return bn_bwd(dz, y, gamma, mean, rstd, dgamma, dbeta, zmask=zmask, inv_loss_scale=inv_loss_scale, accumulate=accumulate,
                   part=part, coef_only=True)
 
@@ -389,13 +407,44 @@
     return (tile_rows.value, ws.value) if ok == 1 else None
 
 
+def conv_c_thin_plan(geom, has_bias=False, sync_stats=False, batch_stats=True):
+    return get_lib().call("sf_conv_c_thin_plan", byref(geom.desc(geom.Ci, geom.Co)), int(bool(has_bias)), int(bool(sync_stats)),
+                          int(bool(batch_stats))) == 1
+
+
+def conv_c_stats(act, wd, geom):
+    assert tuple(act.shape) == geom.in_shape
+    lib = get_lib()
+    d = geom.desc(cl_ld(act), geom.Co)
+    nblk = lib.call("sf_conv_c_rows", byref(d))
+    part = torch.empty((nblk, 2, geom.Co), dtype=torch.float32, device=act.device)
+    lib.call("sf_conv_c_stats", byref(d), act.data_ptr(), wd.data_ptr(), part.data_ptr(), nblk, _stream(act),
+             work=dict(flops=2.0 * rows(act) * geom.Co * geom.Cw, bytes=2.0 * act.numel()))
+    return part
+
+
+def conv_c_tail(act, wd, geom, scale=None, shift=None, relu=False, resid=None, rscale=None, rshift=None, out=None, want_mask=False):
+    assert tuple(act.shape) == geom.in_shape
+    out = cl_empty(geom.out_shape, act.device) if out is None else out
+    assert tuple(out.shape) == geom.out_shape and (resid is None or tuple(resid.shape) == geom.out_shape)
+    M = rows(act)
+    mask = torch.empty((M, geom.Co // 8), dtype=torch.uint8, device=act.device) if want_mask else None
+    get_lib().call("sf_conv_c_tail", byref(geom.desc(cl_ld(act), geom.Co)), act.data_ptr(), wd.data_ptr(), _ptr(scale), _ptr(shift),
+                   _ptr(resid), cl_ld(resid) if resid is not None else 0, _ptr(rscale), _ptr(rshift), int(bool(relu)),
+                   out.data_ptr(), cl_ld(out), _ptr(mask), _stream(act),
+                   work=dict(flops=2.0 * M * geom.Co * geom.Cw,
+                             bytes=2.0 * M * (geom.Ci + geom.Co * (1 + int(resid is not None) + (1 / 16 if want_mask else 0)))))
+    return (out, mask) if want_mask else out
+
+
 def conv_c_bwd(dz, bits, yc, coef, act, wd, geom, dw, bn=None, out_scale=1.0, zero_first=True, out=None):
     plan = conv_c_bwd_plan(geom)
     assert plan is not None, "conv_c_bwd: the planner rejects this geometry"
     tile_rows, ws_bytes = plan
-    assert tuple(act.shape) == geom.in_shape and tuple(dz.shape) == geom.out_shape and tuple(yc.shape) == geom.out_shape
+    assert tuple(act.shape) == geom.in_shape and tuple(dz.shape) == geom.out_shape
+    assert yc is None or tuple(yc.shape) == geom.out_shape
     assert dw.dtype == torch.float32 and dw.is_contiguous() and dw.numel() == geom.Cow * geom.Cw * geom.taps
-    M = rows(yc)
+    M = rows(dz)
     assert bits.dtype == torch.uint8 and bits.is_contiguous() and bits.numel() == M * (geom.Co // 8)
     assert coef.dtype == torch.float32 and coef.is_contiguous() and tuple(coef.shape) == (3, geom.Co)
     d_in = cl_empty(geom.in_shape, dz.device) if out is None else out
@@ -409,12 +458,12 @@
         part = torch.empty((cap, 2, geom.Ci), dtype=torch.float32, device=dz.device)
     ws = _workspace(dz.device, ws_bytes)
     W = 2.0 * M * geom.Co
-    get_lib().call("sf_conv_c_bwd", byref(geom.desc(cl_ld(act), geom.Co)), dz.data_ptr(), cl_ld(dz), bits.data_ptr(), yc.data_ptr(),
-                   cl_ld(yc), coef.data_ptr(), act.data_ptr(), wd.data_ptr(), _ptr(sc), _ptr(sh), _ptr(y0),
+    get_lib().call("sf_conv_c_bwd", byref(geom.desc(cl_ld(act), geom.Co)), dz.data_ptr(), cl_ld(dz), bits.data_ptr(), _ptr(yc),
+                   cl_ld(yc) if yc is not None else 0, coef.data_ptr(), act.data_ptr(), wd.data_ptr(), _ptr(sc), _ptr(sh), _ptr(y0),
                    cl_ld(y0) if y0 is not None else 0, _ptr(part), cap, byref(nrows), d_in.data_ptr(), cl_ld(d_in), dw.data_ptr(),
                    float(out_scale), int(zero_first), ws.data_ptr(), ws.numel(), _stream(dz),
                    work=dict(flops=4.0 * M * geom.Co * geom.Cw,
-                             bytes=W * (2 + 1 / 16) + 2.0 * M * geom.Ci * (2 + int(bn is not None))))
+                             bytes=W * (1 + int(yc is not None) + 1 / 16) + 2.0 * M * geom.Ci * (2 + int(bn is not None))))
     return d_in, (part[:nrows.value] if part is not None and nrows.value > 0 else None)
 
 
```

Measured after the change: 926.1 clips/s (median of 6 runs). +2.5%, better.
